# herobd/handwriting_line_generation

Hardware: AMD Instinct MI355X
Metric: G+D train steps/sec (higher is better)
Workload: dtype f32

## Files before the change

handwriting_line_generation_amd/csrc/conv_mfma.hip:

```cpp
#include "hwg_common.h"
#include "wino_pack.h"
#include <stdlib.h>

namespace {

struct ConvK {
  const float* x;
  const float* w;
  const float* bias;
  float* y;
  int N, H, W, C, K, R, S, sh, sw, ph, pw, dh, dw, P, Q;
  int mode;
  int KN;
  int Pm, Qm;
  int accumulate;
  int ntm;
  int ntm_pad;
  int nsplit;
  float* part;
  int* cnt;
  int dbg;
};

template <int BM, int BN, int BK, int WAVES_M, int WAVES_N, int PF = 1, int WK = 1, bool ABL = false>
// ... 567 lines not shown
    float af[2][PF][MI], bf[2][PF][NI];
    auto lds_group = [&](int g, int slot) {
#pragma unroll
      for (int u = 0; u < PF; ++u) {
        const int kk = kbeg + 2 * (g * PF + u) + lhi;
#pragma unroll
        for (int mi = 0; mi < MI; ++mi) af[slot][u][mi] = Ub[kk * BMU + wm0 + mi * 32 + l31];
#pragma unroll
        for (int ni = 0; ni < NI; ++ni) bf[slot][u][ni] = Vb[kk * BNV + wn0 + ni * 32 + l31];
      }
    };
    lds_group(0, 0);
#pragma unroll
    for (int g = 0; g < NG; ++g) {
      if (g + 1 < NG) lds_group(g + 1, (g + 1) & 1);
      __builtin_amdgcn_sched_barrier(0);
#pragma unroll
      for (int u = 0; u < PF; ++u)
#pragma unroll
        for (int mi = 0; mi < MI; ++mi)
#pragma unroll
          for (int ni = 0; ni < NI; ++ni)
            acc[mi][ni] = __builtin_amdgcn_mfma_f32_32x32x2f32(af[g & 1][u][mi], bf[g & 1][u][ni], acc[mi][ni], 0, 0, 0);
      __builtin_amdgcn_sched_barrier(0);
    }
    if (t + 1 < T) store_tile(buf ^ 1);
    __syncthreads();
  }

  if (do_bias && k0 + tid < a.K) a.part[(long long)blockIdx.x * a.pstride + (long long)RS * a.K * a.C + k0 + tid] = (float)bsum;

  if (WAVES_K > 1) {
    float* red = smem;
#pragma unroll
    for (int mi = 0; mi < MI; ++mi)
#pragma unroll
      for (int ni = 0; ni < NI; ++ni)
#pragma unroll
        for (int e = 0; e < 16; ++e) red[((wid * MI * NI + mi * NI + ni) * 16 + e) * 64 + lane] = acc[mi][ni][e];
    __syncthreads();
    if (wk != 0) return;
#pragma unroll
    for (int mi = 0; mi < MI; ++mi)
#pragma unroll
      for (int ni = 0; ni < NI; ++ni)
#pragma unroll
        for (int e = 0; e < 16; ++e) {
          float sacc = 0.f;
          for (int w = 0; w < WAVES_K; ++w) sacc += red[(((w * WMN + wmn) * MI * NI + mi * NI + ni) * 16 + e) * 64 + lane];
          acc[mi][ni][e] = sacc;
        }
  }

  float* pout = a.part + (long long)blockIdx.x * a.pstride + (long long)tap * a.K * a.C;
#pragma unroll
  for (int mi = 0; mi < MI; ++mi)
#pragma unroll
    for (int e = 0; e < 16; ++e) {
      const int k = k0 + wm0 + mi * 32 + (e & 3) + 8 * (e >> 2) + 4 * lhi;
      if (k >= a.K) continue;
#pragma unroll
      for (int ni = 0; ni < NI; ++ni) {
        const int c = c0 + wn0 + ni * 32 + l31;
        if (TAPN) {
          if (c < RS) pout[(long long)c * a.K + k] = acc[mi][ni][e];
        } else {
          if (c < a.C) pout[(long long)k * a.C + c] = acc[mi][ni][e];
        }
      }
    }
}

__device__ __forceinline__ void wgrad_reduce_vec4_body(const float* __restrict__ part, float* __restrict__ dw, int nsplit, int RS, int S, int K, int C,
                                                       long long sa, long long sb, long long sr, long long ss, int accumulate,
                                                       long long pstride, float* dbias, int bias_accumulate, int bid, int nb) {
  const long long total = (long long)RS * K * C;
  const long long all = total + (dbias ? K : 0);
  const long long n4 = all >> 2;
  for (long long j = bid * (long long)blockDim.x + threadIdx.x; j < n4; j += (long long)nb * blockDim.x) {
    const long long i = j << 2;
    float4 sum = *reinterpret_cast<const float4*>(part + i);
    int sp = 1;
    for (; sp + 3 < nsplit; sp += 4) {
      float4 v[4];
#pragma unroll
      for (int u = 0; u < 4; ++u) v[u] = *reinterpret_cast<const float4*>(part + (long long)(sp + u) * pstride + i);
#pragma unroll
      for (int u = 0; u < 4; ++u) { sum.x += v[u].x; sum.y += v[u].y; sum.z += v[u].z; sum.w += v[u].w; }
    }
    for (; sp < nsplit; ++sp) {
      const float4 v = *reinterpret_cast<const float4*>(part + (long long)sp * pstride + i);
      sum.x += v.x; sum.y += v.y; sum.z += v.z; sum.w += v.w;
    }
    const float e[4] = {sum.x, sum.y, sum.z, sum.w};
    if (i >= total) {
      const int k = (int)(i - total);
#pragma unroll
      for (int u = 0; u < 4; ++u) dbias[k + u] = bias_accumulate ? dbias[k + u] + e[u] : e[u];
      continue;
    }
    const unsigned iu = (unsigned)i, t = iu / (unsigned)C;
    const int c = (int)(iu - t * C);
    const int tap = (int)(t / (unsigned)K);
    const int k = (int)(t - (unsigned)tap * K);
    const long long o = k * sa + c * sb + (tap / S) * sr + (tap % S) * ss;
#pragma unroll
    for (int u = 0; u < 4; ++u) dw[o + u * sb] = accumulate ? dw[o + u * sb] + e[u] : e[u];
  }
}
__global__ __launch_bounds__(256) void wgrad_reduce_kernel(const float* __restrict__ part, float* __restrict__ dw, int nsplit, int RS, int S, int K, int C,
                                                           long long sa, long long sb, long long sr, long long ss, int accumulate,
                                                           long long pstride, float* dbias, int bias_accumulate) {
  wgrad_reduce_vec4_body(part, dw, nsplit, RS, S, K, C, sa, sb, sr, ss, accumulate, pstride, dbias, bias_accumulate, blockIdx.x, gridDim.x);
}
__device__ __forceinline__ void wgrad_reduce_scalar_body(const float* __restrict__ part, float* __restrict__ dw, int nsplit, int RS, int S, int K,
                                                         int C, long long sa, long long sb, long long sr, long long ss, int accumulate,
                                                         long long pstride, float* dbias, int bias_accumulate, int bid, int nb) {
  const long long total = (long long)RS * K * C;
  const long long all = total + (dbias ? K : 0);
  for (long long i = bid * (long long)blockDim.x + threadIdx.x; i < all; i += (long long)nb * blockDim.x) {
    float sum = 0.f;
    for (int sp = 0; sp < nsplit; ++sp) sum += part[(long long)sp * pstride + i];
    if (i >= total) {
      const int k = (int)(i - total);
      dbias[k] = bias_accumulate ? dbias[k] + sum : sum;
      continue;
    }
    const unsigned iu = (unsigned)i, t = iu / (unsigned)C;
    const int c = (int)(iu - t * C);
    const int tap = (int)(t / (unsigned)K);
    const int k = (int)(t - (unsigned)tap * K);
    const long long o = k * sa + c * sb + (tap / S) * sr + (tap % S) * ss;
    dw[o] = accumulate ? dw[o] + sum : sum;
  }
}
__global__ __launch_bounds__(256) void wgrad_reduce_scalar_kernel(const float* __restrict__ part, float* __restrict__ dw, int nsplit, int RS, int S, int K,
                                                                  int C, long long sa, long long sb, long long sr, long long ss, int accumulate,
                                                                  long long pstride, float* dbias, int bias_accumulate) {
  wgrad_reduce_scalar_body(part, dw, nsplit, RS, S, K, C, sa, sb, sr, ss, accumulate, pstride, dbias, bias_accumulate, blockIdx.x, gridDim.x);
}

template <int SL>
__device__ __forceinline__ void wgrad_reduce_lanes_body(const float* part, float* dw, int nsplit, int RS, int S, int K, int C,
                                                        long long sa, long long sb, long long sr, long long ss, int accumulate,
                                                        long long pstride, float* dbias, int bias_accumulate, int bid, float* red) {
  constexpr int OUT = 256 / SL;
  const long long total = (long long)RS * K * C;
  const long long all = total + (dbias ? K : 0);
  const int ol = threadIdx.x % OUT, lane = threadIdx.x / OUT;
  const long long i = (long long)bid * OUT + ol;
  float sum = 0.f;
  if (i < all) {
    int sp = lane;
    for (; sp + 3 * SL < nsplit; sp += 4 * SL) {
      const float v0 = part[(long long)sp * pstride + i], v1 = part[(long long)(sp + SL) * pstride + i];
      const float v2 = part[(long long)(sp + 2 * SL) * pstride + i], v3 = part[(long long)(sp + 3 * SL) * pstride + i];
      sum += v0; sum += v1; sum += v2; sum += v3;
    }
    for (; sp < nsplit; sp += SL) sum += part[(long long)sp * pstride + i];
  }
  red[lane * OUT + ol] = sum;
  __syncthreads();
  if (lane == 0 && i < all) {
    float t = 0.f;
#pragma unroll
    for (int l = 0; l < SL; ++l) t += red[l * OUT + ol];
    if (i >= total) {
      const int kb = (int)(i - total);
      dbias[kb] = bias_accumulate ? dbias[kb] + t : t;
      return;
    }
    const unsigned iu = (unsigned)i, q = iu / (unsigned)C;
    const int c = (int)(iu - q * C);
    const int tap = (int)(q / (unsigned)K);
    const int k = (int)(q - (unsigned)tap * K);
    const long long o = k * sa + c * sb + (tap / S) * sr + (tap % S) * ss;
    dw[o] = accumulate ? dw[o] + t : t;
  }
}
template <int SL>
__global__ __launch_bounds__(256) void wgrad_reduce_lanes_kernel(const float* part, float* dw, int nsplit, int RS, int S, int K, int C,
                                                                 long long sa, long long sb, long long sr, long long ss, int accumulate,
                                                                 long long pstride, float* dbias, int bias_accumulate) {
  __shared__ float red[256];
  wgrad_reduce_lanes_body<SL>(part, dw, nsplit, RS, S, K, C, sa, sb, sr, ss, accumulate, pstride, dbias, bias_accumulate, blockIdx.x, red);
}

template <int SL, int RSC>
__device__ __forceinline__ void wgrad_reduce_rows_body(const float* __restrict__ part, float* __restrict__ dw, int nsplit, int RS_rt, int K, int C,
                                                       long long sa, int accumulate, long long pstride, float* dbias, int bias_accumulate,
                                                       int main_blocks, int bid, float* red) {
  constexpr int KC = 256 / SL;
  const int RS = RSC ? RSC : RS_rt;
  const int ldp = RS | 1;
  const long long KCtot = (long long)K * C;
  if (bid >= main_blocks) {
    const int k = (bid - main_blocks) * 256 + threadIdx.x;
    if (k >= K) return;
    float s = 0.f;
    for (int sp = 0; sp < nsplit; ++sp) s += part[(long long)sp * pstride + RS * KCtot + k];
    dbias[k] = bias_accumulate ? dbias[k] + s : s;
    return;
  }
  const int pl = threadIdx.x % KC, sl = threadIdx.x / KC;
  const long long base = (long long)bid * KC;
  const long long kc = base + pl;
  if (kc < KCtot) {
    if (RSC) {
      float acc[RSC ? RSC : 1];
#pragma unroll
      for (int t = 0; t < RSC; ++t) acc[t] = 0.f;
      for (int sp = sl; sp < nsplit; sp += SL) {
        const float* src = part + (long long)sp * pstride + kc;
#pragma unroll
        for (int t = 0; t < RSC; ++t) acc[t] += src[t * KCtot];
      }
#pragma unroll
      for (int t = 0; t < RSC; ++t) red[(sl * KC + pl) * ldp + t] = acc[t];
    } else {
      for (int t = 0; t < RS; ++t) {
        float a = 0.f;
        for (int sp = sl; sp < nsplit; sp += SL) a += part[(long long)sp * pstride + t * KCtot + kc];
        red[(sl * KC + pl) * ldp + t] = a;
      }
    }
  }
  __syncthreads();
  const int n_out = KC * RS;
  for (int j = threadIdx.x; j < n_out; j += 256) {
    const int p = j / RS, t = j - p * RS;
    const long long q = base + p;
    if (q >= KCtot) break;
    float s = red[p * ldp + t];
#pragma unroll
    for (int l = 1; l < SL; ++l) s += red[(l * KC + p) * ldp + t];
    const long long k = q / C;
    const long long o = k * sa + (q - k * C) * RS + t;
    dw[o] = accumulate ? dw[o] + s : s;
  }
}
template <int SL, int RSC>
__global__ __launch_bounds__(256) void wgrad_reduce_rows_kernel(const float* __restrict__ part, float* __restrict__ dw, int nsplit, int RS_rt, int K, int C,
                                                                long long sa, int accumulate, long long pstride, float* dbias, int bias_accumulate,
                                                                int main_blocks) {
  extern __shared__ float red_rows[];
  wgrad_reduce_rows_body<SL, RSC>(part, dw, nsplit, RS_rt, K, C, sa, accumulate, pstride, dbias, bias_accumulate, main_blocks, blockIdx.x, red_rows);
}

enum { RED_VEC4 = 0, RED_SCALAR = 1, RED_LANES32 = 2, RED_LANES4 = 3, RED_ROWS = 4  };
struct RedEntry {
  const float* part; float* dw; float* dbias;
  long long pstride, sa, sb, sr, ss;
  int nsplit, RS, S, K, C, accumulate, bias_accumulate, variant, first_block, nblocks, main_blocks, tag;
};
constexpr int RED_MAX = 32;
struct RedTable { int n, pad; RedEntry e[RED_MAX]; };

__global__ __launch_bounds__(256) void wgrad_reduce_multi_kernel(const RedTable t) {
  extern __shared__ float red_multi[];
  int lo = 0, hi = t.n - 1;
  while (lo < hi) {
    const int mid = (lo + hi + 1) >> 1;
    if (t.e[mid].first_block <= (int)blockIdx.x) lo = mid; else hi = mid - 1;
  }
  const RedEntry& e = t.e[lo];
  const int bid = (int)blockIdx.x - e.first_block;
  switch (e.variant) {
    case RED_VEC4: wgrad_reduce_vec4_body(e.part, e.dw, e.nsplit, e.RS, e.S, e.K, e.C, e.sa, e.sb, e.sr, e.ss, e.accumulate, e.pstride, e.dbias, e.bias_accumulate, bid, e.nblocks); break;
    case RED_SCALAR: wgrad_reduce_scalar_body(e.part, e.dw, e.nsplit, e.RS, e.S, e.K, e.C, e.sa, e.sb, e.sr, e.ss, e.accumulate, e.pstride, e.dbias, e.bias_accumulate, bid, e.nblocks); break;
    case RED_LANES32: wgrad_reduce_lanes_body<32>(e.part, e.dw, e.nsplit, e.RS, e.S, e.K, e.C, e.sa, e.sb, e.sr, e.ss, e.accumulate, e.pstride, e.dbias, e.bias_accumulate, bid, red_multi); break;
    case RED_LANES4: wgrad_reduce_lanes_body<4>(e.part, e.dw, e.nsplit, e.RS, e.S, e.K, e.C, e.sa, e.sb, e.sr, e.ss, e.accumulate, e.pstride, e.dbias, e.bias_accumulate, bid, red_multi); break;
#define HWG_ROWS_CASE(ID, SL, RSC) \
    case RED_ROWS + ID: wgrad_reduce_rows_body<SL, RSC>(e.part, e.dw, e.nsplit, e.RS, e.K, e.C, e.sa, e.accumulate, e.pstride, e.dbias, e.bias_accumulate, e.main_blocks, bid, red_multi); break;
    HWG_ROWS_CASE(0, 1, 9) HWG_ROWS_CASE(1, 4, 9) HWG_ROWS_CASE(2, 1, 16) HWG_ROWS_CASE(3, 4, 16) HWG_ROWS_CASE(4, 1, 3) HWG_ROWS_CASE(5, 4, 3)
    HWG_ROWS_CASE(6, 1, 0) HWG_ROWS_CASE(7, 4, 0)
#undef HWG_ROWS_CASE
    default: break;
  }
}

__global__ void pack_weight_kernel(const float* src, float* dst, int A, int B, int Bpad, int R, int S,
                                   long long sa, long long sb, long long sr, long long ss, int flip) {
  const long long total = (long long)R * S * A * Bpad;
  for (long long i = blockIdx.x * (long long)blockDim.x + threadIdx.x; i < total; i += (long long)gridDim.x * blockDim.x) {
    const int b = (int)(i % Bpad);
    const long long t = i / Bpad;
    const int aa = (int)(t % A);
    const int tap = (int)(t / A);
    int r = tap / S, s = tap % S;
    if (flip) { r = R - 1 - r; s = S - 1 - s; }
    dst[i] = (b < B) ? src[aa * sa + b * sb + r * sr + s * ss] : 0.f;
  }
}

struct PackEntry {
  const float* src;
  float* dst;
  int A, B, Bpad, R, S, flip;
  long long sa, sb, sr, ss, total, first_block;
  int mode, Apad;
};

constexpr int PACK_PER_BLOCK = 1024;
__global__ __launch_bounds__(256) void pack_weight_multi_kernel(const PackEntry* table, int n) {
  int lo = 0, hi = n - 1;
  while (lo < hi) {
    const int mid = (lo + hi + 1) >> 1;
    if (table[mid].first_block <= (long long)blockIdx.x) lo = mid; else hi = mid - 1;
  }
  const PackEntry e = table[lo];
  const long long base = ((long long)blockIdx.x - e.first_block) * PACK_PER_BLOCK;
#pragma unroll
  for (int j = 0; j < PACK_PER_BLOCK / 256; ++j) {
    const long long i = base + j * 256 + threadIdx.x;
    if (i >= e.total) break;
    if (e.mode == 1) {
      wino_pack_one(e.src, e.dst, i, e.A, e.Apad, e.B, e.Bpad, e.sa, e.sb, e.sr, e.ss, e.flip);
      continue;
    }
    if (e.mode == 2) {
      wino_s2_pack_one(e.src, e.dst, i, e.A, e.B, e.sa, e.sb, e.flip);
      continue;
    }
    const int b = (int)(i % e.Bpad);
    const long long t = i / e.Bpad;
    const int aa = (int)(t % e.A);
    const int tap = (int)(t / e.A);
    int r = tap / e.S, s2 = tap % e.S;
    if (e.flip) { r = e.R - 1 - r; s2 = e.S - 1 - s2; }
    e.dst[i] = (b < e.B) ? e.src[aa * e.sa + b * e.sb + r * e.sr + s2 * e.ss] : 0.f;
  }
}

struct PackEntryS {
  PackEntry e;
  long long dst_off;
  int scale_idx, pad;
};
__global__ __launch_bounds__(256) void pack_weight_multi_scaled_kernel(const PackEntryS* table, int n, float* dst_base, const float* scale_base) {
  int lo = 0, hi = n - 1;
  while (lo < hi) {
    const int mid = (lo + hi + 1) >> 1;
    if (table[mid].e.first_block <= (long long)blockIdx.x) lo = mid; else hi = mid - 1;
  }
  const PackEntry e = table[lo].e;
  float* dst = dst_base + table[lo].dst_off;
  const float sc = scale_base[table[lo].scale_idx];
  const long long base = ((long long)blockIdx.x - e.first_block) * PACK_PER_BLOCK;
#pragma unroll
  for (int j = 0; j < PACK_PER_BLOCK / 256; ++j) {
    const long long i = base + j * 256 + threadIdx.x;
    if (i >= e.total) break;
    if (e.mode == 1) {
      wino_pack_one(e.src, dst, i, e.A, e.Apad, e.B, e.Bpad, e.sa, e.sb, e.sr, e.ss, e.flip, sc);
      continue;
    }
    if (e.mode == 2) {
      wino_s2_pack_one(e.src, dst, i, e.A, e.B, e.sa, e.sb, e.flip, sc);
      continue;
    }
    const int b = (int)(i % e.Bpad);
    const long long t = i / e.Bpad;
    const int aa = (int)(t % e.A);
    const int tap = (int)(t / e.A);
    int r = tap / e.S, s2 = tap % e.S;
    if (e.flip) { r = e.R - 1 - r; s2 = e.S - 1 - s2; }
    dst[i] = (b < e.B) ? __fmul_rn(e.src[aa * e.sa + b * e.sb + r * e.sr + s2 * e.ss], sc) : 0.f;
  }
}

template <int V>
__global__ __launch_bounds__(256) void colsum_partial_kernel(const float* x, long long rows, int C, float* part, long long rows_per_chunk,
                                                             float* direct_out, int accumulate) {
  __shared__ double red[256][V];
  const int cleft = C - (int)blockIdx.y * 64;
  const int cgn = V == 4 ? min(16, (cleft + 3) / 4) : min(64, cleft);
  const int RL = 256 / cgn;
  const int cg = threadIdx.x % cgn, rl = threadIdx.x / cgn;
  const int c = blockIdx.y * 64 + cg * V;
  const long long rb = blockIdx.x * rows_per_chunk;
  const long long re = min(rb + rows_per_chunk, rows);
  double s[V];
#pragma unroll
  for (int e = 0; e < V; ++e) s[e] = 0.0;
  if (rl < RL && c < C) {
    if (V == 4) {
      for (long long rr = rb + rl; rr < re; rr += 4ll * RL) {
        float4 v[4];
#pragma unroll
        for (int u = 0; u < 4; ++u) {
          const long long r2 = rr + (long long)u * RL;
          v[u] = *reinterpret_cast<const float4*>(x + (r2 < re ? r2 : rr) * C + c);
        }
#pragma unroll
        for (int u = 0; u < 4; ++u) {
          if (rr + (long long)u * RL >= re) break;
          s[0] += (double)v[u].x; s[1 % V] += (double)v[u].y; s[2 % V] += (double)v[u].z; s[3 % V] += (double)v[u].w;
        }
      }
    } else {
      for (long long rr = rb + rl; rr < re; rr += RL) s[0] += (double)x[rr * C + c];
    }
  }
#pragma unroll
  for (int e = 0; e < V; ++e) red[threadIdx.x][e] = s[e];
  __syncthreads();
  if ((int)threadIdx.x < min(64, cleft)) {
    const int cc = blockIdx.y * 64 + threadIdx.x;
    double v = 0.0;
    for (int r = 0; r < RL; ++r) v += red[r * cgn + (int)threadIdx.x / V][threadIdx.x % V];
    if (direct_out) direct_out[cc] = accumulate ? direct_out[cc] + (float)v : (float)v;
    else part[(long long)blockIdx.x * C + cc] = (float)v;
  }
}
template <int CC>
__global__ __launch_bounds__(256) void colsum_narrow_kernel(const float* __restrict__ x, long long rows, float* part, long long rows_per_chunk,
                                                            float* direct_out, int accumulate) {
  __shared__ double red[256][CC];
  const long long rb = blockIdx.x * rows_per_chunk;
  const long long re = min(rb + rows_per_chunk, rows);
  double s[CC];
#pragma unroll
  for (int c = 0; c < CC; ++c) s[c] = 0.0;
  for (long long r = rb + threadIdx.x; r < re; r += 256) {
#pragma unroll
    for (int c = 0; c < CC; ++c) s[c] += (double)x[r * CC + c];
  }
#pragma unroll
  for (int c = 0; c < CC; ++c) red[threadIdx.x][c] = s[c];
  __syncthreads();
  for (int w = 128; w >= 1; w >>= 1) {
    if ((int)threadIdx.x < w) {
#pragma unroll
      for (int c = 0; c < CC; ++c) red[threadIdx.x][c] += red[threadIdx.x + w][c];
    }
    __syncthreads();
  }
  if ((int)threadIdx.x < CC) {
    const float v = (float)red[0][threadIdx.x];
    if (direct_out) direct_out[threadIdx.x] = accumulate ? direct_out[threadIdx.x] + v : v;
    else part[(long long)blockIdx.x * CC + threadIdx.x] = v;
  }
}
__global__ __launch_bounds__(256) void colsum_final_kernel(const float* part, int chunks, int C, float* out, int accumulate) {
  __shared__ float red[16][17];
  const int cl = threadIdx.x & 15, lane = threadIdx.x >> 4;
  const int c = blockIdx.x * 16 + cl;
  float s = 0.f;
  if (c < C)
    for (int i = lane; i < chunks; i += 16) s += part[(long long)i * C + c];
  red[lane][cl] = s;
  __syncthreads();
  if (lane == 0 && c < C) {
    float t = 0.f;
#pragma unroll
    for (int l = 0; l < 16; ++l) t += red[l][cl];
    out[c] = accumulate ? out[c] + t : t;
  }
}

template <int BM, int BN, int BK, int WM_, int WN_>
void launch_conv(const ConvK& k, dim3 grid, hipStream_t st, int pf) {
  if constexpr (BM == 64 && BN == 64) {
    if (hwg_tune().conv_wk >= 2) {
      hipLaunchKernelGGL((conv_mfma_kernel<BM, BN, BK, WM_, WN_, 3, 2>), grid, dim3(128 * WM_ * WN_), 0, st, k);
      return;
    }
  }
  if constexpr (BM == 128 && BN == 128 && BK == 32) {
    if (k.dbg) { hipLaunchKernelGGL((conv_mfma_kernel<BM, BN, BK, WM_, WN_, 3, 1, true>), grid, dim3(64 * WM_ * WN_), 0, st, k); return; }
  }
  if (pf >= 3) hipLaunchKernelGGL((conv_mfma_kernel<BM, BN, BK, WM_, WN_, 3>), grid, dim3(64 * WM_ * WN_), 0, st, k);
  else if (pf == 2) hipLaunchKernelGGL((conv_mfma_kernel<BM, BN, BK, WM_, WN_, 2>), grid, dim3(64 * WM_ * WN_), 0, st, k);
  else hipLaunchKernelGGL((conv_mfma_kernel<BM, BN, BK, WM_, WN_, 1>), grid, dim3(64 * WM_ * WN_), 0, st, k);
}

struct WgPlan {
  int cfg;
  int bmu, bnv, bkp;
  int tiles_u, tiles_v, nsplit, chunk;
};
static void wg_split(WgPlan& p, long long Mtot, long long ns) {
  const long long max_ns = (Mtot + 4LL * p.bkp - 1) / (4LL * p.bkp);
  if (ns > max_ns) ns = max_ns;
  if (ns < 1) ns = 1;
  long long chunk = (Mtot + ns - 1) / ns;
  chunk = (chunk + p.bkp - 1) / p.bkp * p.bkp;
  ns = (Mtot + chunk - 1) / chunk;
  if (ns < 1) ns = 1;
  p.nsplit = (int)ns;
  p.chunk = (int)chunk;
}
static void wg_tile(WgPlan& p, int cfg, int K, int C) {
  p.cfg = cfg;
  if (cfg == 0) { p.bmu = 128; p.bnv = 128; p.bkp = 32; }
  else if (cfg == 1) { p.bmu = 64; p.bnv = 64; p.bkp = 32; }
  else { p.bmu = 32; p.bnv = 32; p.bkp = 32; }
  p.tiles_u = hwg_cdiv(K, p.bmu);
  p.tiles_v = hwg_cdiv(C, p.bnv);
}
static WgPlan plan_wgrad_model(const hwg_conv_desc* d);
WgPlan plan_wgrad(const hwg_conv_desc* d) {
  static thread_local HwgPlanCache<WgPlan> cache;
  return cache.get(d, plan_wgrad_model);
}
static WgPlan plan_wgrad_model(const hwg_conv_desc* d) {
  WgPlan p;
  const int K = d->K, C = d->C;
  const long long Mtot = (long long)d->N * d->P * d->Q;
  if (K <= 32 && C <= 32) {
    wg_tile(p, 2, K, C);
    const long long base = (long long)d->R * d->S * p.tiles_u * p.tiles_v;
    wg_split(p, Mtot, (1024 + base - 1) / base);
    return p;
  }
  if (const char* f = hwg_tune().wgrad_force; *f) {
    int fc = -1, ft = 0;
    if (sscanf(f, "%d,%d", &fc, &ft) == 2 && ft > 0 && (fc == 1 || (fc == 0 && K >= 128 && C >= 128))) {
      wg_tile(p, fc, K, C);
      const long long base = (long long)d->R * d->S * p.tiles_u * p.tiles_v;
      wg_split(p, Mtot, (ft + base - 1) / base);
      return p;
    }
  }
  static const int splits[14] = {1, 2, 3, 4, 6, 8, 12, 16, 24, 32, 48, 64, 96, 128};
  static const double tflops[2] = {106.0, 90.0}, overhead[2] = {1.0, 1.0};
  static const int waves_per_block[2] = {16, 8};
  const double wbytes = 4.0 * d->R * d->S * K * C;
  double best = 1e30;
  WgPlan bp = p;
  for (int cfg = (K >= 128 && C >= 128) ? 0 : 1; cfg <= 1; ++cfg) {
    WgPlan c;
    wg_tile(c, cfg, K, C);
    const double base = (double)d->R * d->S * c.tiles_u * c.tiles_v;
    int last_ns = 0;
    for (int si = 0; si < 14; ++si) {
      wg_split(c, Mtot, splits[si]);
      if (c.nsplit == last_ns) continue;
      last_ns = c.nsplit;
      if (wbytes * c.nsplit > 2.0e9) break;
      const double q = base * c.nsplit / 256.0;
      const double quanta = q <= 2.0 ? ceil(q) : q + 0.5;
      double resident = (q > 1.0 ? q : 1.0);
      const double max_blocks = 32.0 / waves_per_block[cfg];
      if (resident > max_blocks) resident = max_blocks;
      resident *= waves_per_block[cfg];
      const double rate = tflops[cfg] * (0.65 + 0.35 * (resident >= 24.0 ? 1.0 : resident / 24.0));
      const double step_s = 2.0 * c.bmu * c.bnv * c.bkp / (rate * 1e12 / 256.0);
      const double tm = quanta * ((double)c.chunk / c.bkp + overhead[cfg]) * step_s + (c.nsplit + 1) * wbytes / 8.0e12 + 3e-6;
      if (tm < best) { best = tm; bp = c; }
    }
  }
  return bp;
}

}

extern "C" int hwg_conv_pack_weight(const float* src, float* dst, int A, int B, int Bpad, int R, int S,
                                    long long sa, long long sb, long long sr, long long ss, int flip, void* stream) {
  HWG_REQUIRE(src && dst && A > 0 && B > 0 && Bpad >= B && R > 0 && S > 0, "conv_pack_weight: bad arguments");
  const long long total = (long long)R * S * A * Bpad;
  hipLaunchKernelGGL(pack_weight_kernel, dim3(hwg_stream_grid(total, 256)), dim3(256), 0, (hipStream_t)stream,
                     src, dst, A, B, Bpad, R, S, sa, sb, sr, ss, flip);
  HWG_LAUNCH_CHECK("conv_pack_weight");
  return HWG_OK;
}

extern "C" int hwg_conv_pack_weight_multi(const void* table, int n_entries, long long total_blocks, void* stream) {
  HWG_REQUIRE(table && n_entries > 0 && total_blocks > 0 && total_blocks < (1LL << 31), "conv_pack_weight_multi: bad arguments");
  hipLaunchKernelGGL(pack_weight_multi_kernel, dim3((unsigned)total_blocks), dim3(256), 0, (hipStream_t)stream, (const PackEntry*)table, n_entries);
  HWG_LAUNCH_CHECK("conv_pack_weight_multi");
  return HWG_OK;
}

extern "C" int hwg_conv_pack_weight_multi_scaled(const void* table, int n_entries, long long total_blocks, float* dst_base, const float* scale_base,
                                                 void* stream) {
  HWG_REQUIRE(table && dst_base && scale_base && n_entries > 0 && total_blocks > 0 && total_blocks < (1LL << 31), "conv_pack_weight_multi_scaled: bad arguments");
  hipLaunchKernelGGL(pack_weight_multi_scaled_kernel, dim3((unsigned)total_blocks), dim3(256), 0, (hipStream_t)stream, (const PackEntryS*)table, n_entries,
                     dst_base, scale_base);
  HWG_LAUNCH_CHECK("conv_pack_weight_multi_scaled");
  return HWG_OK;
}

int hwg_conv_c1_fwd_impl(const hwg_conv_desc* d, const float* x, const float* w, const float* bias, float* y, int accumulate, hipStream_t st);
int hwg_conv_to1_fwd_impl(const hwg_conv_desc* d, const float* x, const float* w, const float* bias, float* y, int accumulate, hipStream_t st);
int hwg_conv_wgrad_direct_impl(const hwg_conv_desc* d, const float* u, const float* v, float* dw, long long sa, long long sb,
                               long long sr, long long ss, int accumulate, void* ws, size_t ws_bytes, hipStream_t st);
size_t hwg_conv_wgrad_direct_workspace(const hwg_conv_desc* d);

static int check_desc(const hwg_conv_desc* d, const char* who) {
  HWG_REQUIRE(d, "%s: null descriptor", who);
  HWG_REQUIRE(d->N > 0 && d->H > 0 && d->W > 0 && d->C > 0 && d->K > 0 && d->R > 0 && d->S > 0 && d->P > 0 && d->Q > 0,
              "%s: non-positive dimension", who);
  HWG_REQUIRE(d->stride_h > 0 && d->stride_w > 0 && d->dil_h > 0 && d->dil_w > 0, "%s: bad stride/dilation", who);
  return HWG_OK;
}

int hwg_conv_split_reduce_launch(const float* part, const float* bias, float* y, long long total, int K, int nsplit, int accumulate, hipStream_t st) {
  hipLaunchKernelGGL(conv_split_reduce_kernel, dim3(hwg_stream_grid(total / 4 + 1, 256)), dim3(256), 0, st, part, bias, y, total, K, nsplit, accumulate);
  HWG_LAUNCH_CHECK("conv_split_reduce");
  return HWG_OK;
}

struct ConvPlan {
  bool mfma;
  int bm, bn, bk, nsplit, classes;
  long long Mc;
  int merged, KN, Pm, Qm;
  double model_s;
};
static ConvPlan plan_conv_model(const hwg_conv_desc* d);
static ConvPlan plan_conv(const hwg_conv_desc* d) {
  static thread_local HwgPlanCache<ConvPlan> cache;
  return cache.get(d, plan_conv_model);
}
static ConvPlan plan_conv_model(const hwg_conv_desc* d) {
  ConvPlan p;
  p.mfma = !((!d->transposed) && (d->K <= 2 || d->C == 1));
  p.classes = d->transposed ? d->stride_h * d->stride_w : 1;
  p.Mc = (long long)d->N * d->P * d->Q;
  if (d->transposed) p.Mc = (long long)d->N * hwg_cdiv(d->P, d->stride_h) * hwg_cdiv(d->Q, d->stride_w);
  p.merged = 0; p.KN = d->K; p.Pm = p.Qm = 0;
  if (d->transposed && p.classes > 1 && d->R % d->stride_h == 0 && d->S % d->stride_w == 0 &&
      (hwg_tune().conv_merge == 2 || (hwg_tune().conv_merge == 1 && d->K < 32))) {
    for (int c = 0; c < d->stride_h; ++c) p.Pm = std::max(p.Pm, hwg_cdiv(d->P - c, d->stride_h) + (c + d->pad_h) / d->stride_h);
    for (int c = 0; c < d->stride_w; ++c) p.Qm = std::max(p.Qm, hwg_cdiv(d->Q - c, d->stride_w) + (c + d->pad_w) / d->stride_w);
    p.merged = 1; p.KN = p.classes * d->K; p.Mc = (long long)d->N * p.Pm * p.Qm; p.classes = 1;
  }
  const int bk = (d->C % 32 == 0) ? 32 : 16;
  const int taps_total = d->R * d->S;
  const double taps_per_class = (double)taps_total / (d->transposed ? d->stride_h * d->stride_w : 1);
  const double T_total = taps_per_class * (d->C / bk);
  const int min_taps = d->transposed ? (d->R / d->stride_h) * (d->S / d->stride_w) : taps_total;
  const int min_steps = (min_taps > 0 ? min_taps : 1) * (d->C / bk);
  const double out_bytes = 4.0 * d->N * d->P * d->Q * d->K;
  struct Tile { int bm, bn; double tflops, overhead; };
  static const Tile tiles[4] = {{128, 128, 108.0, 1.0}, {128, 64, 94.0, 1.25}, {64, 64, 88.0, 1.5}, {128, 32, 62.0, 1.5}};
  static const int splits[8] = {1, 2, 3, 4, 6, 8, 12, 16};
  int bm = 128, bn = 32, ns = 1;
  double best = 1e30;
  for (int ti = 0; ti < 4; ++ti) {
    const Tile& t = tiles[ti];
    if (p.KN <= 32 ? t.bn != 32 : (t.bn == 32 || (t.bn == 128 && p.KN < 96))) continue;
    const double step_s = 2.0 * t.bm * t.bn * bk / (t.tflops * 1e12 / 256.0);
    const double per_xcd = (double)hwg_cdiv(hwg_cdiv(p.Mc, t.bm), 8) * hwg_cdiv(p.KN, t.bn) * p.classes;
    for (int si = 0; si < 8; ++si) {
      const int n = splits[si];
      if (n > 1 && (min_steps / n < 3 || out_bytes * n > 1.5e9)) break;
      const double q = per_xcd * n / 32.0;
      const double quanta = q <= 8.0 ? ceil(q) : q + 0.5;
// ... 727 lines not shown
```

handwriting_line_generation_amd/csrc/conv_wino.hip:

```cpp
#include "hwg_common.h"
#include "wino_pack.h"
#include <stdlib.h>

namespace {

struct WinoK {
  const float* x;
  const float* u;
  const float* bias;
  float* y;
  int N, H, W, C, K, Kpad, P, Q, ph, pw, TP, TQ;
  int M;
  int accumulate;
  int nsplit;
  float* part;
  int* cnt;
  int mt, nt;
  int xcd_order;
  int bal;
  int bal_tile0;
  int mt_edge;
  int dbg;
  int x_img, x_row, x_pix, x_tc, x_run;
  int y_img, y_row, y_pix, y_kc, y_run;
// ... 1137 lines not shown
  }
  if (!direct && a.cnt) {
    __shared__ int last_flag;
    if (hwg_split_arrive_block(a.cnt + slot_id, pieces, &last_flag)) {
      const long long total = (long long)a.N * a.P * a.Q * a.K;
      const int k = n0 + (tid & 63);
      const float bl = (a.bias && k < a.K) ? a.bias[k] : 0.f;
      auto finish = [&](long long o) {
        float v = BAL ? 0.f : hwg_load_agent(a.part + o);
        for (int sp = BAL ? 0 : 1; sp < pieces; ++sp) v += hwg_load_agent(a.part + sp * total + o);
        if (a.bias) v += bl;
        if (a.accumulate) v += a.y[o];
        a.y[o] = v;
      };
      if constexpr (MT == 2) {
        for (int tile = tid >> 6; tile < 64; tile += 8) {
          const int base = tile_out[tile], ext = tile_ext[tile];
          if (base < 0 || k >= a.K) continue;
          const long long ob = (long long)base * a.K + k;
#pragma unroll
          for (int i = 0; i < 2; ++i) {
            if (i && !(ext & 1)) continue;
#pragma unroll
            for (int j = 0; j < 2; ++j) {
              if (j && !(ext & 2)) continue;
              finish(ob + (i * a.Q + j) * a.K);
            }
          }
        }
      } else {
        const long long kch = (long long)(k / a.y_kc) * a.y_run + (k % a.y_kc);
        for (int tile = tid >> 6; tile < 64; tile += 8) {
          const int base = tile_out[tile], ext = tile_ext[tile];
          if (base < 0 || k >= a.K) continue;
          for (int i = 0; i < (ext & 3); ++i)
            for (int j = 0; j < (ext >> 2); ++j) finish((long long)base + (long long)i * a.y_row + (long long)j * a.y_pix + kch);
        }
      }
    }
  }
  if (!BAL || whole) break;
  unit += t1 - t0;
  if (unit >= unit_end) break;
  __syncthreads();
  }
}


constexpr int WINO_DB = 4;

__global__ __launch_bounds__(768) void wino_conv_big_kernel(WinoK a) {
  constexpr int TM = 64, TN = 64, NX = 256;
  constexpr int PSV = TM * 16 + 8, PSU = TN * 16 + 8;
  constexpr int VBUF = 4 * PSV, UBUF = 4 * PSU;
  constexpr int DA = WINO_DB;
  constexpr int XI = TM * 16 / NX;
  constexpr int UD = TN / 16;
  __shared__ __attribute__((aligned(16))) float smem[2 * VBUF + DA * UBUF];
  float* const Vs = smem;
  float* const Us = smem + 2 * VBUF;

  const int tid = threadIdx.x, lane = tid & 63, wid = tid >> 6;
  int mtile, ntile, split;
  if (!wino_work_item(a, mtile, ntile, split)) return;
  const int m0 = mtile * TM;
  const int n0 = ntile * TN;
  const int T_all = a.C >> 4;
  const int t0 = (int)((long long)T_all * split / a.nsplit);
  const int t1 = (int)((long long)T_all * (split + 1) / a.nsplit);
  const int S = 4 * (t1 - t0);
  const int TC = t1 - t0;
  const int rot = TC > 0 ? (int)(((unsigned)mtile * 7u + (unsigned)ntile * 3u) % (unsigned)TC) : 0;
  auto chunk_of = [&](int tau) { int c = tau + rot; if (c >= TC) c -= TC; return t0 + c; };

  if (wid >= 8) {
    const int pt = tid - 512;
    const int pw = wid - 8;
    int x_off[XI], x_ok[XI];
    const int xb = pt & 3, xc4 = (pt >> 2) & 3;
    const int x_lds0 = xb * PSV + swz(pt >> 4, xc4);
    const float x_sa = (xb == 3) ? -1.f : 1.f, x_sb = (xb & 1) ? 1.f : -1.f;
    const int row_stride = a.W * a.C;
#pragma unroll
    for (int it = 0; it < XI; ++it) {
      const int b = xb, c4 = xc4, row = (pt >> 4) + 16 * it;
      const int m = m0 + row;
      const bool mok = m < a.M;
      const int mm = mok ? m : 0;
      const int tj = mm % a.TQ;
      const int t2 = mm / a.TQ;
      const int ti = t2 % a.TP;
      const int n = t2 / a.TP;
      const int w = 2 * tj - a.pw + b;
      const bool wok = mok && w >= 0 && w < a.W;
      const int h0 = 2 * ti - a.ph;
      x_off[it] = ((n * a.H + h0) * a.W + (wok ? w : 0)) * a.C + c4 * 4;
      int okm = 0;
#pragma unroll
      for (int r = 0; r < 4; ++r)
        if (wok && h0 + r >= 0 && h0 + r < a.H) okm |= 1 << r;
      x_ok[it] = okm;
    }
    int u_src[UD];
#pragma unroll
    for (int i = 0; i < UD; ++i) {
      const int row = 16 * i + (lane >> 2), slot = lane & 3;
      int k = n0 + row;
      if (k >= a.Kpad) k = a.Kpad - 1;
      u_src[i] = (pw * a.Kpad + k) * 16 + 4 * (slot ^ ((row >> 1) & 3));
    }
    const long long u_round = 4LL * a.Kpad * 16;
    float4 raw[XI][4], tr[XI][4];
    auto load_x = [&](int t) {
#pragma unroll
      for (int it = 0; it < XI; ++it)
#pragma unroll
        for (int r = 0; r < 4; ++r) {
          const int off = (x_ok[it] >> r) & 1 ? x_off[it] + r * row_stride + t * 16 : 0;
          raw[it][r] = *reinterpret_cast<const float4*>(a.x + off);
        }
    };
    auto col_transform = [&]() {
#pragma unroll
      for (int it = 0; it < XI; ++it) {
        float4 d[4];
#pragma unroll
        for (int r = 0; r < 4; ++r) {
          d[r] = raw[it][r];
          if (!((x_ok[it] >> r) & 1)) d[r] = make_float4(0.f, 0.f, 0.f, 0.f);
        }
        tr[it][0] = make_float4(d[0].x - d[2].x, d[0].y - d[2].y, d[0].z - d[2].z, d[0].w - d[2].w);
        tr[it][1] = make_float4(d[1].x + d[2].x, d[1].y + d[2].y, d[1].z + d[2].z, d[1].w + d[2].w);
        tr[it][2] = make_float4(d[2].x - d[1].x, d[2].y - d[1].y, d[2].z - d[1].z, d[2].w - d[1].w);
        tr[it][3] = make_float4(d[1].x - d[3].x, d[1].y - d[3].y, d[1].z - d[3].z, d[1].w - d[3].w);
      }
    };
    auto dma_u = [&](int ring, int round) {
      const float* base = a.u + (long long)round * u_round;
      float* dst = Us + ring * UBUF + pw * PSU;
#pragma unroll
      for (int i = 0; i < UD; ++i)
        __builtin_amdgcn_global_load_lds((const __attribute__((address_space(1))) void*)(base + u_src[i]),
                                         (__attribute__((address_space(3))) void*)(dst + i * 256), 16, 0, 0);
    };
    auto write_v = [&](int buf, int r) {
      float* B = Vs + buf * VBUF;
#pragma unroll
      for (int it = 0; it < XI; ++it) {
        const float4 v = tr[it][r];
        float4 o;
        o.x = x_sa * v.x + x_sb * quad_partner(v.x);
        o.y = x_sa * v.y + x_sb * quad_partner(v.y);
        o.z = x_sa * v.z + x_sb * quad_partner(v.z);
        o.w = x_sa * v.w + x_sb * quad_partner(v.w);
        *reinterpret_cast<float4*>(B + x_lds0 + it * 256) = o;
      }
    };
    int hist[DA], hdma[DA];
#pragma unroll
    for (int j = 0; j < DA; ++j) { hist[j] = 0; hdma[j] = 0; }
    int issued = 0;
    if (S > 0) {
      load_x(chunk_of(0));
      col_transform();
      write_v(0, 0);
    }
    for (; issued < DA && issued < S; ++issued) dma_u(issued, 4 * chunk_of(issued >> 2) + (issued & 3));
    wait_vmcnt((issued - 1) * UD);
#pragma unroll
    for (int j = 0; j < DA; ++j) { hdma[j] = j < issued ? UD : 0; hist[j] = hdma[j]; }
    __syncthreads();
    int ring = 0;
    for (int t = t0; t < t1; ++t) {
#pragma unroll
      for (int r = 0; r < 4; ++r) {
        const int s = 4 * (t - t0) + r;
        int ops = 0, dops = 0;
        if (s >= 1 && issued < S) { dma_u(ring, 4 * chunk_of(issued >> 2) + (issued & 3)); ++issued; ring = ring == DA - 1 ? 0 : ring + 1; ops = dops = UD; }
        if (s + 1 < S) {
          if (r == 3) col_transform();
          write_v((r + 1) & 1, (r + 1) & 3);
          if (r == 1 && t + 1 < t1) { load_x(chunk_of(t + 1 - t0)); ops += XI * 4; }
        }
#pragma unroll
        for (int j = 0; j + 1 < DA; ++j) { hist[j] = hist[j + 1]; hdma[j] = hdma[j + 1]; }
        hist[DA - 1] = ops; hdma[DA - 1] = dops;
        if (s + 1 < S) {
          int back = issued - 2 - s;
          int n = 0, seen = 0;
#pragma unroll
          for (int j = DA - 1; j >= 0; --j) {
            if (seen < back || (seen == back && hdma[j] == 0)) { n += hist[j]; seen += hdma[j] ? 1 : 0; }
            else if (seen == back && hdma[j] != 0) { n += hist[j] - hdma[j]; seen = back + 1; }
          }
          wait_vmcnt(n);
        }
        __syncthreads();
      }
    }
    return;
  }

  const int cm = wid >> 2, cn = wid & 3;
  const int frow = lane & 15, fchunk = lane >> 4;
  const int a_off0 = swz(cm * 32 + frow, fchunk);
  const int a_off1 = swz(cm * 32 + 16 + frow, fchunk);
  const int b_off = swz(cn * 16 + frow, fchunk);

  f32x4 acc[16][2];
#pragma unroll
  for (int p = 0; p < 16; ++p) {
    acc[p][0] = (f32x4){0.f, 0.f, 0.f, 0.f};
    acc[p][1] = (f32x4){0.f, 0.f, 0.f, 0.f};
  }
  __syncthreads();
  int ring = 0;
  for (int t = t0; t < t1; ++t) {
#pragma unroll
    for (int r = 0; r < 4; ++r) {
      const float* A = Vs + (r & 1) * VBUF;
      const float* B = Us + ring * UBUF + b_off;
      ring = ring == DA - 1 ? 0 : ring + 1;
      float4 fa0[2], fa1[2], fb[2];
      fa0[0] = *reinterpret_cast<const float4*>(A + a_off0);
      fa1[0] = *reinterpret_cast<const float4*>(A + a_off1);
      fb[0] = *reinterpret_cast<const float4*>(B);
#pragma unroll
      for (int pb = 0; pb < 4; ++pb) {
        const int c = pb & 1;
        if (pb < 3) {
          fa0[c ^ 1] = *reinterpret_cast<const float4*>(A + (pb + 1) * PSV + a_off0);
          fa1[c ^ 1] = *reinterpret_cast<const float4*>(A + (pb + 1) * PSV + a_off1);
          fb[c ^ 1] = *reinterpret_cast<const float4*>(B + (pb + 1) * PSU);
        }
        __builtin_amdgcn_sched_barrier(0);
        f32x4& c0 = acc[r * 4 + pb][0];
        f32x4& c1 = acc[r * 4 + pb][1];
        c0 = __builtin_amdgcn_mfma_f32_16x16x4f32(fa0[c].x, fb[c].x, c0, 0, 0, 0);
        c1 = __builtin_amdgcn_mfma_f32_16x16x4f32(fa1[c].x, fb[c].x, c1, 0, 0, 0);
        c0 = __builtin_amdgcn_mfma_f32_16x16x4f32(fa0[c].y, fb[c].y, c0, 0, 0, 0);
        c1 = __builtin_amdgcn_mfma_f32_16x16x4f32(fa1[c].y, fb[c].y, c1, 0, 0, 0);
        c0 = __builtin_amdgcn_mfma_f32_16x16x4f32(fa0[c].z, fb[c].z, c0, 0, 0, 0);
        c1 = __builtin_amdgcn_mfma_f32_16x16x4f32(fa1[c].z, fb[c].z, c1, 0, 0, 0);
        c0 = __builtin_amdgcn_mfma_f32_16x16x4f32(fa0[c].w, fb[c].w, c0, 0, 0, 0);
        c1 = __builtin_amdgcn_mfma_f32_16x16x4f32(fa1[c].w, fb[c].w, c1, 0, 0, 0);
        __builtin_amdgcn_sched_barrier(0);
      }
      __syncthreads();
    }
  }

  const int k = n0 + cn * 16 + (lane & 15);
  const bool direct = a.nsplit == 1;
  float* yg = direct ? a.y : a.part + (long long)split * ((long long)a.N * a.P * a.Q * a.K);
  const float bv = (direct && a.bias && k < a.K) ? a.bias[k] : 0.f;
  const bool accum = direct && a.accumulate;
#pragma unroll
  for (int blk = 0; blk < 2; ++blk)
#pragma unroll
    for (int e = 0; e < 4; ++e) {
      const int m = m0 + cm * 32 + blk * 16 + (lane >> 4) * 4 + e;
      if (m >= a.M || k >= a.K) continue;
      const int tj = m % a.TQ;
      const int t2 = m / a.TQ;
      const int ti = t2 % a.TP;
      const int n = t2 / a.TP;
      float mm[16];
#pragma unroll
      for (int p = 0; p < 16; ++p) mm[p] = acc[p][blk][e];
#pragma unroll
      for (int j = 0; j < 4; ++j) {
        const float s0 = mm[0 * 4 + j] + mm[1 * 4 + j] + mm[2 * 4 + j];
        const float s1 = mm[1 * 4 + j] - mm[2 * 4 + j] - mm[3 * 4 + j];
        mm[0 * 4 + j] = s0;
        mm[1 * 4 + j] = s1;
      }
#pragma unroll
      for (int i = 0; i < 2; ++i) {
        const int p = 2 * ti + i;
        if (p >= a.P) continue;
        const float y0 = mm[i * 4 + 0] + mm[i * 4 + 1] + mm[i * 4 + 2];
        const float y1 = mm[i * 4 + 1] - mm[i * 4 + 2] - mm[i * 4 + 3];
#pragma unroll
        for (int j = 0; j < 2; ++j) {
          const int q = 2 * tj + j;
          if (q >= a.Q) continue;
          const long long o = (((long long)n * a.P + p) * a.Q + q) * a.K + k;
          float v = (j == 0 ? y0 : y1) + bv;
          if (accum) v += yg[o];
          yg[o] = v;
        }
      }
    }
}

__global__ __launch_bounds__(256) void wino_pack_weight_kernel(const float* src, float* dst, int A, int Apad, int B, int Bpad,
                                                               long long sa, long long sb, long long sr, long long ss, int flip) {
  const long long total = (long long)Apad * Bpad;
  for (long long i = blockIdx.x * (long long)blockDim.x + threadIdx.x; i < total; i += (long long)gridDim.x * blockDim.x)
    wino_pack_one(src, dst, i, A, Apad, B, Bpad, sa, sb, sr, ss, flip);
}

template <int VEC>
__global__ __launch_bounds__(256) void wino_bal_reduce_kernel(WinoK a, int T_all) {
  const int KV = a.K / VEC;
  const int total = a.N * a.P * a.Q * KV;
  const long long plane = (long long)a.N * a.P * a.Q * a.K;
  const int U_bal = (a.mt * a.nt - a.bal_tile0) * T_all;
  const int e = a.mt_edge;
  for (int i = blockIdx.x * blockDim.x + threadIdx.x; i < total; i += gridDim.x * blockDim.x) {
    const int k = (i % KV) * VEC, pix = i / KV;
    const int q = pix % a.Q, t = pix / a.Q, p = t % a.P, n = t / a.P;
    const int m = (n * a.TP + p / e) * a.TQ + q / e;
    const int rel = (m >> 6) + a.mt * (k >> 6) - a.bal_tile0;
    if (rel < 0) continue;
    const int g_first = wino_bal_owner(a.bal, U_bal, rel * T_all), g_last = wino_bal_owner(a.bal, U_bal, rel * T_all + T_all - 1);
    if (g_first == g_last) continue;
    const long long o = (long long)n * a.y_img + (long long)p * a.y_row + (long long)q * a.y_pix + (long long)(k / a.y_kc) * a.y_run + k % a.y_kc;
    float s[VEC];
#pragma unroll
    for (int v = 0; v < VEC; ++v) s[v] = 0.f;
    for (int j = 0; j <= g_last - g_first; ++j) {
      if constexpr (VEC == 4) {
        const float4 v = *reinterpret_cast<const float4*>(a.part + j * plane + o);
        s[0] += v.x; s[1] += v.y; s[2] += v.z; s[3] += v.w;
      } else {
        s[0] += a.part[j * plane + o];
      }
    }
#pragma unroll
    for (int v = 0; v < VEC; ++v) {
      if (a.bias) s[v] += a.bias[k + v];
      if (a.accumulate) s[v] += a.y[o + v];
    }
    if constexpr (VEC == 4) *reinterpret_cast<float4*>(a.y + o) = make_float4(s[0], s[1], s[2], s[3]);
    else a.y[o] = s[0];
  }
}

struct WinoPlan {
  int cfg;
  int tm, tn, nsplit;
  int bal, bal_tile0, bal_pieces;
  int bal_segs, bal_cut, bal_cut_pieces;
  double model_s;
};
static void wino_cfg(WinoPlan& p, int cfg) {
  static const int tms[8] = {64, 32, 128, 64, 32, 64, 64, 32}, tns[8] = {32, 64, 16, 32, 64, 64, 64, 32};
  p.cfg = cfg; p.tm = tms[cfg]; p.tn = tns[cfg];
  p.bal = p.bal_tile0 = p.bal_pieces = p.bal_segs = p.bal_cut = p.bal_cut_pieces = 0;
}
static bool wino_balance(WinoPlan& p, long long tiles, int chunks, int g_force = 0, int a_force = -1) {
  const long long lead = a_force >= 0 ? (long long)a_force : tiles / 256 * 256;
  const long long rem = tiles - lead;
  if (lead % 256 || rem <= 0 || (g_force <= 0 && rem >= 240)) return false;
  const long long units = rem * chunks;
  long long G = g_force > 0 ? g_force : (units < 256 ? units : 256);
  if (G > units) G = units;
  if (G < 1 || (g_force <= 0 && G <= rem) || units * G >= (1ll << 31) || units >= (1ll << 24)) return false;
  p.bal = (int)G; p.bal_tile0 = (int)lead; p.nsplit = 1;
  p.bal_pieces = 1; p.bal_segs = 1; p.bal_cut = 0; p.bal_cut_pieces = 0;
  for (long long t = 0; t < rem; ++t) {
    const int n = wino_bal_owner((int)G, (int)units, (int)(t * chunks + chunks - 1)) - wino_bal_owner((int)G, (int)units, (int)(t * chunks)) + 1;
    if (n > p.bal_pieces) p.bal_pieces = n;
    if (n > 1) { ++p.bal_cut; p.bal_cut_pieces += n; }
  }
  for (long long g = 0; g < G; ++g) {
    const long long u0 = units * g / G, u1 = units * (g + 1) / G;
    if (u1 > u0) p.bal_segs = std::max(p.bal_segs, (int)((u1 - 1) / chunks - u0 / chunks + 1));
  }
  return true;
}
struct WinoCost { int cfg; double fixed_us, step_us; };
static const WinoCost kWinoCost[6] = {{1, 2.5, 1.17}, {5, 11.0, 2.09}, {0, 8.0, 1.2}, {2, 6.5, 1.5}, {6, 15.7, 1.04}, {7, 2.0, 1.0}};
static WinoPlan plan_wino_model(const hwg_conv_desc* d);
static WinoPlan plan_wino(const hwg_conv_desc* d, double* model_s = nullptr) {
  static thread_local HwgPlanCache<WinoPlan> cache;
  const WinoPlan p = cache.get(d, plan_wino_model);
  if (model_s) *model_s = p.model_s;
  return p;
}
static WinoPlan plan_wino_model(const hwg_conv_desc* d) {
  WinoPlan best;
  wino_cfg(best, d->K <= 16 ? 2 : d->K <= 48 ? 0 : 1);
  best.nsplit = 1;
  const long long M = (long long)d->N * hwg_cdiv(d->P, 2) * hwg_cdiv(d->Q, 2);
  const int chunks = d->C / 16;
  const double out_bytes = 4.0 * d->N * d->P * d->Q * d->K;
  double best_t = 1e30;
  WinoCost cost6 = kWinoCost[4];
  if (const char* e = hwg_tune().wino_cost6; *e) { double f = 0, s2 = 0; if (sscanf(e, "%lf,%lf", &f, &s2) == 2) { cost6.fixed_us = f; cost6.step_us = s2; } }
  for (int ci = 0; ci < 6; ++ci) {
    const WinoCost& wc = ci == 4 ? cost6 : kWinoCost[ci];
    if (wc.cfg == 7 && (d->K <= 16 || d->K > 64)) continue;
    if (wc.cfg == 2 && d->K > 16) continue;
    if (wc.cfg == 0 && d->K > 48) continue;
    if ((wc.cfg == 1 || wc.cfg == 5 || wc.cfg == 6) && d->K <= 48) continue;
    if (wc.cfg == 5 && d->C < 64) continue;
    WinoPlan p;
    wino_cfg(p, wc.cfg);
    const long long blocks = (long long)hwg_cdiv(M, p.tm) * hwg_cdiv(d->K, p.tn);
    for (int ns = 1; ns <= 8 && ns * 2 <= (chunks > 1 ? chunks : 2); ns *= 2) {
      if (ns > 1 && (chunks / ns < 2 || out_bytes * ns > 1.5e9)) break;
      const double q = (double)(blocks * ns) / 256.0;
      const double rounds = q <= 3.0 ? (double)hwg_cdiv(blocks * ns, 256) : q + 0.5;
      double t = rounds * (wc.fixed_us + 4.0 * hwg_cdiv(chunks, ns) * wc.step_us) * 1e-6;
      if (ns > 1) t += (ns + 1) * out_bytes / 3.0e12 + 6e-6;
      if (t < best_t) { best_t = t; best = p; best.nsplit = ns; }
    }
  }
  const int bal_mode = hwg_tune().wino_bal[0] ? atoi(hwg_tune().wino_bal) : 0;
  if (d->K > 48 && bal_mode >= 0 && !hwg_tune().w64_nodma && !(hwg_tune().conv_dbg & 512) && (long long)d->N * d->P * d->Q * d->K < (1ll << 31)) {
    WinoPlan p;
    wino_cfg(p, 6);
    const long long tiles = (long long)hwg_cdiv(M, 64) * hwg_cdiv(d->K, 64);
    int gf = 0, af = -1;
    if (bal_mode > 0) sscanf(hwg_tune().wino_bal, "%d,%d", &gf, &af);
    if (wino_balance(p, tiles, chunks, gf, af) && (p.bal_pieces <= 1 || (double)p.bal_pieces * out_bytes <= 1.5e9)) {
      const long long units = (tiles - p.bal_tile0) * chunks;
      const long long c = hwg_cdiv(units, (long long)p.bal);
      double t = (p.bal_tile0 / 256) * (cost6.fixed_us + 4.0 * chunks * cost6.step_us) * 1e-6;
      t += (double)hwg_cdiv((long long)p.bal, 256ll) * (cost6.fixed_us - 4.0 + (p.bal_segs - 1) * 5.0 + 4.0 * c * cost6.step_us) * 1e-6;
      if (p.bal_cut) t += (p.bal_cut_pieces + p.bal_cut) * (out_bytes / tiles) / 3.0e12 + out_bytes / 2.0e13 + 6e-6;
      if (bal_mode > 0 || t < 0.97 * best_t) { best = p; best_t = t; }
    }
  }
  if (const char* f = hwg_tune().wino_force; *f) {
    int fc = -1, fs = 0;
    const int n = sscanf(f, "%d,%d", &fc, &fs);
    if (n >= 1 && fc >= 0 && fc <= 7 && fc != 3 && fc != 4 && (fc == 2 || d->K > 16)) { const int ns = best.nsplit; wino_cfg(best, fc); best.nsplit = ns; }
    if (n >= 2 && fs >= 1) best.nsplit = fs > chunks ? chunks : fs;
  }
  best.model_s = best_t;
  return best;
}

}

extern "C" int hwg_wino_supported(const hwg_conv_desc* d) {
  if (!d || d->transposed) return 0;
  if (d->R != 3 || d->S != 3 || d->stride_h != 1 || d->stride_w != 1 || d->dil_h != 1 || d->dil_w != 1) return 0;
  if (d->C % 16 != 0 || d->K < 16) return 0;
  if (d->P != d->H + 2 * d->pad_h - 2 || d->Q != d->W + 2 * d->pad_w - 2) return 0;
  return hwg_tune().wino == 0 ? 0 : 1;
}

double hwg_conv_direct_model_seconds(const hwg_conv_desc* d);

extern "C" int hwg_wino_preferred(const hwg_conv_desc* d) {
  if (!hwg_wino_supported(d)) return 0;
  if (hwg_tune().wino == 2) return 1;
  double tw = 0.0;
  (void)plan_wino(d, &tw);
  return tw < 0.97 * hwg_conv_direct_model_seconds(d) ? 1 : 0;
}

extern "C" size_t hwg_wino_weight_floats(int A, int B) {
  const size_t Apad = (size_t)(A + 15) / 16 * 16, Bpad = (size_t)(B + 15) / 16 * 16;
  return 16 * Apad * Bpad;
}

extern "C" int hwg_wino_pack_weight(const float* src, float* dst, int A, int B, long long sa, long long sb, long long sr, long long ss,
                                    int flip, void* stream) {
  HWG_REQUIRE(src && dst && A > 0 && B > 0, "wino_pack_weight: bad arguments");
  const int Apad = (A + 15) / 16 * 16, Bpad = (B + 15) / 16 * 16;
  hipLaunchKernelGGL(wino_pack_weight_kernel, dim3(hwg_stream_grid((long long)Apad * Bpad, 256)), dim3(256), 0, (hipStream_t)stream, src, dst, A, Apad,
                     B, Bpad, sa, sb, sr, ss, flip);
  HWG_LAUNCH_CHECK("wino_pack_weight");
  return HWG_OK;
}

extern "C" size_t hwg_wino_conv_workspace(const hwg_conv_desc* d) {
  if (!hwg_wino_supported(d)) return 0;
  const WinoPlan p = plan_wino(d);
  if (p.bal > 0) return p.bal_pieces > 1 ? (size_t)p.bal_pieces * d->N * d->P * d->Q * d->K * sizeof(float) : 0;
  if (p.nsplit <= 1) return 0;
  return (size_t)p.nsplit * d->N * d->P * d->Q * d->K * sizeof(float);
}

int hwg_conv_split_reduce_launch(const float* part, const float* bias, float* y, long long total, int K, int nsplit, int accumulate, hipStream_t st);

extern "C" int hwg_wino_conv_fwd(const hwg_conv_desc* d, const float* x, const float* u, const float* bias, float* y, int accumulate,
                                 void* workspace, size_t workspace_bytes, void* stream) {
  HWG_REQUIRE(d && x && u && y, "wino_conv_fwd: null pointer");
  HWG_REQUIRE(hwg_wino_supported(d), "wino_conv_fwd: needs a 3x3 stride-1 dilation-1 convolution with C %% 16 == 0 and K >= 16");
  hipStream_t st = (hipStream_t)stream;
  const WinoPlan p = plan_wino(d);
  const size_t need = hwg_wino_conv_workspace(d);
  if (need && (!workspace || workspace_bytes < need)) {
    hwg_set_error("wino_conv_fwd: workspace too small (%zu < %zu)", workspace_bytes, need);
    return HWG_ERR_WORKSPACE;
  }
  WinoK k;
  k.x = x; k.u = u; k.bias = bias; k.y = y;
  k.N = d->N; k.H = d->H; k.W = d->W; k.C = d->C; k.K = d->K; k.Kpad = (d->K + 15) / 16 * 16;
  k.P = d->P; k.Q = d->Q; k.ph = d->pad_h; k.pw = d->pad_w;
  k.TP = hwg_cdiv(d->P, 2); k.TQ = hwg_cdiv(d->Q, 2);
  k.M = d->N * k.TP * k.TQ;
  k.accumulate = accumulate;
  k.nsplit = p.nsplit;
  k.part = (float*)workspace;
  k.mt = hwg_cdiv(k.M, p.tm); k.nt = hwg_cdiv(d->K, p.tn);
  k.xcd_order = hwg_tune().wino_order;
  k.bal = p.bal; k.bal_tile0 = p.bal_tile0;
  k.mt_edge = 2; k.dbg = hwg_tune().conv_dbg;
  k.x_img = k.x_row = k.x_pix = k.x_tc = k.x_run = 0;
  k.y_img = d->P * d->Q * d->K; k.y_row = d->Q * d->K; k.y_pix = d->K; k.y_kc = d->K; k.y_run = 0;
  dim3 grid(p.bal > 0 ? p.bal_tile0 + (p.bal + 7) / 8 * 8 : (k.mt * k.nt * p.nsplit + 7) / 8 * 8);
  k.cnt = nullptr;
  const bool counted = p.cfg == 0 || p.cfg == 1 || p.cfg == 2 || p.cfg == 7 || (p.cfg == 6 && !hwg_tune().w64_nodma && !(hwg_tune().conv_dbg & 512));
  if ((p.bal > 0 ? p.bal_pieces > 1 : p.nsplit > 1) && counted && hwg_tune().split_inkernel && (long long)k.mt * k.nt * 8 <= HWG_SPLIT_COUNTERS) {
    k.cnt = hwg_split_counters(st);
    if (!k.cnt) return HWG_ERR_LAUNCH;
  }
  const int prof = hwg_prof_open(HWG_PROF_CONV_WINO, 2.0 * d->N * d->P * d->Q * (double)d->K * d->C * 9.0, st);
  if (p.cfg == 0) hipLaunchKernelGGL((wino_conv_kernel<4, 2>), grid, dim3(512), 0, st, k);
  else if (p.cfg == 1) hipLaunchKernelGGL((wino_conv_kernel<2, 4>), grid, dim3(512), 0, st, k);
  else if (p.cfg == 2) hipLaunchKernelGGL((wino_conv_kernel<8, 1>), grid, dim3(512), 0, st, k);
  else if (p.cfg == 7) hipLaunchKernelGGL((wino_conv_kernel<2, 2>), grid, dim3(256), 0, st, k);
  else if (p.cfg == 5) hipLaunchKernelGGL(wino_conv_big_kernel, grid, dim3(768), 0, st, k);
  else if (p.cfg == 6 && !hwg_tune().w64_nodma && (hwg_tune().conv_dbg & 512)) hipLaunchKernelGGL((wino_conv64d_kernel<1, false>), grid, dim3(512), 0, st, k);
  else if (p.cfg == 6 && !hwg_tune().w64_nodma && p.bal > 0) hipLaunchKernelGGL((wino_conv64d_kernel<0, true>), grid, dim3(512), 0, st, k);
  else if (p.cfg == 6 && !hwg_tune().w64_nodma) hipLaunchKernelGGL((wino_conv64d_kernel<0, false>), grid, dim3(512), 0, st, k);
  else if (p.cfg == 6) hipLaunchKernelGGL(wino_conv64_kernel, grid, dim3(512), 0, st, k);
  else hipLaunchKernelGGL((wino_conv_ws_kernel<1, 4>), grid, dim3(512), 0, st, k);
  hwg_prof_close(prof, st);
  hwg_note_plan(HWG_PROF_CONV_WINO, p.cfg, p.bal > 0 ? -p.bal : p.nsplit);
  HWG_LAUNCH_CHECK("wino_conv_fwd");
  if (k.cnt) {
  } else if (p.bal > 0 && p.bal_pieces > 1) {
    const long long total = (long long)d->N * d->P * d->Q * d->K;
    const double cut = (double)(k.mt * k.nt - p.bal_tile0) / (k.mt * k.nt);
    const int prof2 = hwg_prof_open(HWG_PROF_CONV_REDUCE, 4.0 * total * cut * (p.bal_pieces + 1), st);
    const int vec = d->K % 4 == 0 ? 4 : 1;
    const dim3 rgrid(hwg_stream_grid(total / vec, 256));
    if (vec == 4) hipLaunchKernelGGL(wino_bal_reduce_kernel<4>, rgrid, dim3(256), 0, st, k, d->C / 16);
    else hipLaunchKernelGGL(wino_bal_reduce_kernel<1>, rgrid, dim3(256), 0, st, k, d->C / 16);
    hwg_prof_close(prof2, st);
    HWG_LAUNCH_CHECK("wino_bal_reduce");
  } else if (p.nsplit > 1) {
    const long long total = (long long)d->N * d->P * d->Q * d->K;
    const int prof2 = hwg_prof_open(HWG_PROF_CONV_REDUCE, 4.0 * total * (p.nsplit + 1), st);
    const int rc = hwg_conv_split_reduce_launch((const float*)workspace, bias, y, total, d->K, p.nsplit, accumulate, st);
    hwg_prof_close(prof2, st);
    if (rc) return rc;
  }
  return HWG_OK;
}


namespace {

struct S2Geom {
  int N, Hv, Wv, Cv, Kv, Pv, Qv, pad;
  int x_img, x_row, x_pix, x_tc, x_run, y_img, y_row, y_pix, y_kc, y_run;
  double flops;
};

bool s2_geom(const hwg_conv_desc* d, S2Geom& g) {
  if (!d || d->R != 4 || d->S != 4 || d->stride_h != 2 || d->stride_w != 2 || d->pad_h || d->pad_w || d->dil_h != 1 || d->dil_w != 1) return false;
  if (d->C % 16 || d->K % 4 || d->N < 1 || d->H < 1 || d->W < 1) return false;
  const long long in_e = (long long)d->N * d->H * d->W * d->C, out_e = (long long)d->N * d->P * d->Q * d->K;
  if (in_e >= (1ll << 31) || out_e >= (1ll << 31)) return false;
  g.N = d->N;
  if (!d->transposed) {
    if (d->H < 4 || d->W < 4 || d->P != (d->H - 4) / 2 + 1 || d->Q != (d->W - 4) / 2 + 1) return false;
    g.Hv = d->P + 1; g.Wv = d->Q + 1; g.Cv = 4 * d->C; g.Kv = d->K; g.Pv = d->P; g.Qv = d->Q; g.pad = 0;
    g.x_img = d->H * d->W * d->C; g.x_row = 2 * d->W * d->C; g.x_pix = 2 * d->C; g.x_tc = 2 * d->C / 16; g.x_run = d->W * d->C;
    g.y_img = d->P * d->Q * d->K; g.y_row = d->Q * d->K; g.y_pix = d->K; g.y_kc = d->K; g.y_run = 0;
    g.flops = 2.0 * d->N * d->P * d->Q * (double)d->K * d->C * 16.0;
  } else {
    if (d->P != 2 * d->H + 2 || d->Q != 2 * d->W + 2) return false;
    g.Hv = d->H; g.Wv = d->W; g.Cv = d->C; g.Kv = 4 * d->K; g.Pv = d->H + 1; g.Qv = d->W + 1; g.pad = 1;
    g.x_img = d->H * d->W * d->C; g.x_row = d->W * d->C; g.x_pix = d->C; g.x_tc = d->C / 16; g.x_run = 0;
    g.y_img = d->P * d->Q * d->K; g.y_row = 2 * d->Q * d->K; g.y_pix = 2 * d->K; g.y_kc = 2 * d->K; g.y_run = d->Q * d->K;
    g.flops = 2.0 * d->N * d->H * d->W * (double)d->K * d->C * 16.0;
  }
  return g.Kv > 48;
}

WinoPlan plan_wino_s2_model(const hwg_conv_desc* d) {
  WinoPlan best;
  wino_cfg(best, 6);
  best.nsplit = 1;
  best.model_s = 1e30;
  S2Geom g;
  if (!s2_geom(d, g)) return best;
  const long long M = (long long)g.N * hwg_cdiv(g.Pv, 3) * hwg_cdiv(g.Qv, 3);
  const int chunks = g.Cv / 16;
  const double out_bytes = 4.0 * g.N * g.Pv * g.Qv * g.Kv;
  const WinoCost wc = kWinoCost[4];
  const long long tiles = (long long)hwg_cdiv(M, 64) * hwg_cdiv(g.Kv, 64);
  double best_t = 1e30;
  for (int ns = 1; ns <= 8 && ns * 2 <= (chunks > 1 ? chunks : 2); ns *= 2) {
    if (ns > 1 && (chunks / ns < 2 || out_bytes * ns > 1.5e9)) break;
    const double q = (double)(tiles * ns) / 256.0;
    const double rounds = q <= 3.0 ? (double)hwg_cdiv(tiles * ns, 256) : q + 0.5;
    double t = rounds * (wc.fixed_us + 4.0 * hwg_cdiv(chunks, ns) * wc.step_us) * 1e-6;
    if (ns > 1) t += (ns + 1) * out_bytes / 3.0e12 + 6e-6;
    if (t < best_t) { best_t = t; best.nsplit = ns; }
  }
  const int bal_mode = hwg_tune().wino_bal[0] ? atoi(hwg_tune().wino_bal) : 0;
  if (bal_mode >= 0) {
    WinoPlan p;
    wino_cfg(p, 6);
    int gf = 0, af = -1;
    if (bal_mode > 0) sscanf(hwg_tune().wino_bal, "%d,%d", &gf, &af);
    if (wino_balance(p, tiles, chunks, gf, af) && (p.bal_pieces <= 1 || (double)p.bal_pieces * out_bytes <= 1.5e9)) {
      const long long units = (tiles - p.bal_tile0) * chunks;
      const long long c = hwg_cdiv(units, (long long)p.bal);
      double t = (p.bal_tile0 / 256) * (wc.fixed_us + 4.0 * chunks * wc.step_us) * 1e-6;
      t += (double)hwg_cdiv((long long)p.bal, 256ll) * (wc.fixed_us - 4.0 + (p.bal_segs - 1) * 5.0 + 4.0 * c * wc.step_us) * 1e-6;
      if (p.bal_cut) t += (p.bal_cut_pieces + p.bal_cut) * (out_bytes / tiles) / 3.0e12 + out_bytes / 2.0e13 + 6e-6;
      if (bal_mode > 0 || t < 0.97 * best_t) { best = p; best_t = t; }
    }
  }
  if (const char* f = hwg_tune().wino_force; *f) {
    int fc = -1, fs = 0;
    if (sscanf(f, "%d,%d", &fc, &fs) >= 2 && fs >= 1) { const int keep = fs > chunks ? chunks : fs; wino_cfg(best, 6); best.nsplit = keep; }
  }
  best.model_s = best_t;
  return best;
}
WinoPlan plan_wino_s2(const hwg_conv_desc* d) {
  static thread_local HwgPlanCache<WinoPlan> cache;
  return cache.get(d, plan_wino_s2_model);
}

__global__ __launch_bounds__(256) void wino_s2_pack_kernel(const float* src, float* dst, int Kc, int Cc, long long sk, long long sc, int dgrad, long long total) {
  for (long long i = blockIdx.x * (long long)blockDim.x + threadIdx.x; i < total; i += (long long)gridDim.x * blockDim.x)
    wino_s2_pack_one(src, dst, i, Kc, Cc, sk, sc, dgrad);
}

}

extern "C" int hwg_wino_s2_supported(const hwg_conv_desc* d) {
  S2Geom g;
  return hwg_tune().wino_s2 != 0 && !hwg_tune().w64_nodma && s2_geom(d, g) ? 1 : 0;
}

extern "C" int hwg_wino_s2_preferred(const hwg_conv_desc* d) {
  if (!hwg_wino_s2_supported(d)) return 0;
  if (hwg_tune().wino_s2 == 2) return 1;
  const WinoPlan p = plan_wino_s2(d);
  return p.model_s < 0.9 * hwg_conv_direct_model_seconds(d) ? 1 : 0;
}

extern "C" size_t hwg_wino_s2_weight_floats(int Kc, int Cc, int dgrad) {
  const size_t A = dgrad ? 4 * (size_t)Cc : (size_t)Kc, B = dgrad ? (size_t)Kc : 4 * (size_t)Cc;
  return 16 * ((A + 15) / 16 * 16) * ((B + 15) / 16 * 16);
}

extern "C" int hwg_wino_s2_pack_weight(const float* src, float* dst, int Kc, int Cc, long long sk, long long sc, int dgrad, void* stream) {
  HWG_REQUIRE(src && dst && Kc > 0 && Cc > 0, "wino_s2_pack_weight: bad arguments");
  const long long total = (long long)hwg_wino_s2_weight_floats(Kc, Cc, dgrad) / 16;
  hipLaunchKernelGGL(wino_s2_pack_kernel, dim3(hwg_stream_grid(total, 256)), dim3(256), 0, (hipStream_t)stream, src, dst, Kc, Cc, sk, sc, dgrad, total);
  HWG_LAUNCH_CHECK("wino_s2_pack_weight");
  return HWG_OK;
}

extern "C" size_t hwg_wino_s2_workspace(const hwg_conv_desc* d) {
  if (!hwg_wino_s2_supported(d)) return 0;
  const WinoPlan p = plan_wino_s2(d);
  const size_t out = (size_t)d->N * d->P * d->Q * d->K * sizeof(float);
  if (p.bal > 0) return p.bal_pieces > 1 ? p.bal_pieces * out : 0;
  return p.nsplit > 1 ? p.nsplit * out : 0;
}

extern "C" int hwg_wino_s2_conv(const hwg_conv_desc* d, const float* x, const float* u, const float* bias, float* y, int accumulate,
                                void* workspace, size_t workspace_bytes, void* stream) {
  HWG_REQUIRE(d && x && u && y, "wino_s2_conv: null pointer");
  S2Geom g;
  HWG_REQUIRE(hwg_wino_s2_supported(d) && s2_geom(d, g), "wino_s2_conv: needs a 4x4 stride-2 pad-0 convolution (or its data gradient) with C %% 16 == 0");
  HWG_REQUIRE(!(d->transposed && bias), "wino_s2_conv: the data-gradient form takes no bias");
  hipStream_t st = (hipStream_t)stream;
  const WinoPlan p = plan_wino_s2(d);
  const size_t need = hwg_wino_s2_workspace(d);
  if (need && (!workspace || workspace_bytes < need)) {
    hwg_set_error("wino_s2_conv: workspace too small (%zu < %zu)", workspace_bytes, need);
    return HWG_ERR_WORKSPACE;
  }
  WinoK k;
  k.x = x; k.u = u; k.bias = bias; k.y = y;
  k.N = g.N; k.H = g.Hv; k.W = g.Wv; k.C = g.Cv; k.K = g.Kv; k.Kpad = (g.Kv + 15) / 16 * 16;
  k.P = g.Pv; k.Q = g.Qv; k.ph = g.pad; k.pw = g.pad;
  k.TP = hwg_cdiv(g.Pv, 3); k.TQ = hwg_cdiv(g.Qv, 3);
  k.M = g.N * k.TP * k.TQ;
  k.accumulate = accumulate;
  k.nsplit = p.nsplit;
  k.part = (float*)workspace;
  k.mt = hwg_cdiv(k.M, 64); k.nt = hwg_cdiv(g.Kv, 64);
  k.xcd_order = hwg_tune().wino_order;
  k.bal = p.bal; k.bal_tile0 = p.bal_tile0;
  k.mt_edge = 3; k.dbg = 0;
  k.x_img = g.x_img; k.x_row = g.x_row; k.x_pix = g.x_pix; k.x_tc = g.x_tc; k.x_run = g.x_run;
  k.y_img = g.y_img; k.y_row = g.y_row; k.y_pix = g.y_pix; k.y_kc = g.y_kc; k.y_run = g.y_run;
  dim3 grid(p.bal > 0 ? p.bal_tile0 + (p.bal + 7) / 8 * 8 : (k.mt * k.nt * p.nsplit + 7) / 8 * 8);
  k.cnt = nullptr;
  if ((p.bal > 0 ? p.bal_pieces > 1 : p.nsplit > 1) && hwg_tune().split_inkernel && (long long)k.mt * k.nt <= HWG_SPLIT_COUNTERS) {
    k.cnt = hwg_split_counters(st);
    if (!k.cnt) return HWG_ERR_LAUNCH;
  }
  const int prof = hwg_prof_open(HWG_PROF_CONV_WINO, g.flops, st);
  if (p.bal > 0) hipLaunchKernelGGL((wino_conv64d_kernel<0, true, 3>), grid, dim3(512), 0, st, k);
  else hipLaunchKernelGGL((wino_conv64d_kernel<0, false, 3>), grid, dim3(512), 0, st, k);
  hwg_prof_close(prof, st);
  hwg_note_plan(HWG_PROF_CONV_WINO, 36, p.bal > 0 ? -p.bal : p.nsplit);
  HWG_LAUNCH_CHECK("wino_s2_conv");
  const long long total = (long long)d->N * d->P * d->Q * d->K;
  if (k.cnt) {
  } else if (p.bal > 0 && p.bal_pieces > 1) {
    const double cut = (double)(k.mt * k.nt - p.bal_tile0) / (k.mt * k.nt);
    const int prof2 = hwg_prof_open(HWG_PROF_CONV_REDUCE, 4.0 * total * cut * (p.bal_pieces + 1), st);
    hipLaunchKernelGGL(wino_bal_reduce_kernel<4>, dim3(hwg_stream_grid(total / 4, 256)), dim3(256), 0, st, k, g.Cv / 16);
    hwg_prof_close(prof2, st);
    HWG_LAUNCH_CHECK("wino_bal_reduce");
  } else if (p.bal <= 0 && p.nsplit > 1) {
    const int prof2 = hwg_prof_open(HWG_PROF_CONV_REDUCE, 4.0 * total * (p.nsplit + 1), st);
    const int rc = hwg_conv_split_reduce_launch((const float*)workspace, bias, y, total, d->K, p.nsplit, accumulate, st);
    hwg_prof_close(prof2, st);
    if (rc) return rc;
  }
  return HWG_OK;
}

extern "C" int hwg_wino_conv_describe(const hwg_conv_desc* d, int* out) {
  HWG_REQUIRE(d && out, "wino_conv_describe: null pointer");
  for (int i = 0; i < 8; ++i) out[i] = -1;
  WinoPlan p;
  long long tiles;
  int chunks;
  S2Geom g;
  if (d->R == 4 && d->S == 4) {
    if (!hwg_wino_s2_supported(d) || !s2_geom(d, g)) return HWG_OK;
    p = plan_wino_s2(d);
    tiles = (long long)hwg_cdiv((long long)g.N * hwg_cdiv(g.Pv, 3) * hwg_cdiv(g.Qv, 3), 64ll) * hwg_cdiv(g.Kv, 64);
    chunks = g.Cv / 16;
  } else {
    if (!hwg_wino_supported(d)) return HWG_OK;
    p = plan_wino(d);
    tiles = (long long)hwg_cdiv((long long)d->N * hwg_cdiv(d->P, 2) * hwg_cdiv(d->Q, 2), (long long)p.tm) * hwg_cdiv(d->K, p.tn);
    chunks = d->C / 16;
  }
  out[0] = p.cfg; out[1] = p.nsplit; out[2] = p.bal; out[3] = p.bal_tile0; out[4] = p.bal > 0 ? p.bal_pieces : (p.nsplit > 1 ? p.nsplit : 1);
  out[5] = (int)tiles; out[6] = chunks; out[7] = p.bal > 0 ? p.bal_segs : 1;
  return HWG_OK;
}
```

handwriting_line_generation_amd/csrc/seq_ops.hip:

```cpp
#include "hwg_common.h"

namespace {

__global__ __launch_bounds__(256) void log_softmax_fwd_kernel(const float* x, float* y, long long rows, int C, int Bn, int Tn, int transpose) {
  const int lane = threadIdx.x & 63;
  const long long wave = (blockIdx.x * 256LL + threadIdx.x) >> 6;
  const long long nw = (gridDim.x * 256LL) >> 6;
  for (long long r = wave; r < rows; r += nw) {
    const float* xr = x + r * C;
    float m = -INFINITY;
    for (int c = lane; c < C; c += 64) m = fmaxf(m, xr[c]);
    m = wave_max(m);
    float s = 0.f;
    for (int c = lane; c < C; c += 64) s += expf(xr[c] - m);
    s = wave_sum(s);
    const float lse = m + logf(s);
    long long orow = r;
    if (transpose) { const long long b = r / Tn, t = r % Tn; orow = t * Bn + b; }
    float* yr = y + orow * C;
    for (int c = lane; c < C; c += 64) yr[c] = xr[c] - lse;
  }
}
__global__ __launch_bounds__(256) void log_softmax_bwd_kernel(const float* dy, const float* y, float* dx, long long rows, int C, int Bn, int Tn,
                                                              int transpose) {
  const int lane = threadIdx.x & 63;
  const long long wave = (blockIdx.x * 256LL + threadIdx.x) >> 6;
  const long long nw = (gridDim.x * 256LL) >> 6;
  for (long long r = wave; r < rows; r += nw) {
    long long orow = r;
    if (transpose) { const long long b = r / Tn, t = r % Tn; orow = t * Bn + b; }
    const float* dyr = dy + orow * C;
    const float* yr = y + orow * C;
    float s = 0.f;
    for (int c = lane; c < C; c += 64) s += dyr[c];
    s = wave_sum(s);
    float* dxr = dx + r * C;
    for (int c = lane; c < C; c += 64) dxr[c] = dyr[c] - expf(yr[c]) * s;
  }
}

__device__ __forceinline__ int ctc_ext(const int* tg, int s) { return (s & 1) ? tg[s >> 1] : 0; }

__device__ __forceinline__ void ctc_alpha_body(float* rows , int b, const float* lp,
                                               const int* targets, const int* in_len, const int* tg_len, int T, int B, int C, int Lmax,
                                               float* log_alpha, float* nll) {
  const int S = tg_len[b];
  const int Tb = in_len[b];
  const int NS = 2 * S + 1;
  const int NSmax = 2 * Lmax + 1;
  const int* tg = targets + (long long)b * Lmax;
  float* la = log_alpha + (long long)b * T * NSmax;
  int* ext = (int*)(rows + 2 * NSmax);
  const float NEG = -INFINITY;
  for (int s = threadIdx.x; s < NSmax; s += 256) {
    float v = NEG;
    if (Tb > 0) {
      if (s == 0) v = lp[((long long)0 * B + b) * C + 0];
      else if (s == 1 && S > 0) v = lp[((long long)0 * B + b) * C + tg[0]];
    }
    la[s] = v;
    rows[s] = v;
    ext[s] = s < NS ? ctc_ext(tg, s) : 0;
  }
  __syncthreads();
  for (int t = 1; t < Tb; ++t) {
    const float* prev = rows + ((t - 1) & 1) * NSmax;
    float* cur = rows + (t & 1) * NSmax;
    for (int s = threadIdx.x; s < NSmax; s += 256) {
      float v = NEG;
      if (s < NS) {
        const int cs = ext[s];
        const float l = lp[((long long)t * B + b) * C + cs];
        const float la1 = prev[s];
        float lamax = la1;
        float la2 = NEG, la3 = NEG;
        if (s > 0) { la2 = prev[s - 1]; if (la2 > lamax) lamax = la2; }
        if (s > 1 && ext[s - 2] != cs) { la3 = prev[s - 2]; if (la3 > lamax) lamax = la3; }
        if (lamax == NEG) lamax = 0.f;
        v = logf(expf(la1 - lamax) + expf(la2 - lamax) + expf(la3 - lamax)) + lamax + l;
      }
      cur[s] = v;
      la[(long long)t * NSmax + s] = v;
    }
    __syncthreads();
  }
  if (threadIdx.x == 0) {
    float r;
    if (Tb <= 0) r = (S == 0) ? 0.f : INFINITY;
    else {
      const float* last = rows + ((Tb - 1) & 1) * NSmax;
      const float l1 = last[NS - 1];
      const float l2 = (S > 0) ? last[NS - 2] : NEG;
      float m = fmaxf(l1, l2);
      if (m == NEG) m = 0.f;
      r = -(logf(expf(l1 - m) + expf(l2 - m)) + m);
    }
    nll[b] = r;
  }
}
__global__ __launch_bounds__(256) void ctc_alpha_kernel(const float* lp, const int* targets, const int* in_len, const int* tg_len, int T, int B,
                                                        int C, int Lmax, float* log_alpha, float* nll) {
  extern __shared__ float rows[];
  ctc_alpha_body(rows, blockIdx.x, lp, targets, in_len, tg_len, T, B, C, Lmax, log_alpha, nll);
}
__global__ void ctc_mean_kernel(const float* nll, const int* tg_len, int B, float* loss, int* finite_flag) {
  if (threadIdx.x == 0 && blockIdx.x == 0) {
    float s = 0.f;
    for (int b = 0; b < B; ++b) { const int l = tg_len[b] > 1 ? tg_len[b] : 1; s += nll[b] / (float)l; }
    s /= (float)B;
    const int inf = isinf(s) ? 1 : 0;
    *finite_flag = inf ? 0 : 1;
    *loss = inf ? 0.f : s;
  }
}
__device__ __forceinline__ void ctc_beta_body(float* rows , int b, const float* lp,
                                              const int* targets, const int* in_len, const int* tg_len, int T, int B, int C, int Lmax,
                                              float* log_beta) {
  const int S = tg_len[b];
  const int Tb = in_len[b];
  const int NS = 2 * S + 1;
  const int NSmax = 2 * Lmax + 1;
  const int* tg = targets + (long long)b * Lmax;
  float* lb = log_beta + (long long)b * T * NSmax;
  int* ext = (int*)(rows + 2 * NSmax);
  const float NEG = -INFINITY;
  for (int s = threadIdx.x; s < NSmax; s += 256) ext[s] = s < NS ? ctc_ext(tg, s) : 0;
  __syncthreads();
  if (Tb <= 0) return;
  for (int t = Tb - 1; t >= 0; --t) {
    float* cur = rows + (t & 1) * NSmax;
    const float* nxt = rows + ((t + 1) & 1) * NSmax;
    for (int s = threadIdx.x; s < NSmax; s += 256) {
      float v = NEG;
      if (s < NS) {
        const int cs = ext[s];
        const float l = lp[((long long)t * B + b) * C + cs];
        if (t == Tb - 1) {
          if (s == NS - 1 || (S > 0 && s == NS - 2)) v = l;
        } else {
          const float lb1 = nxt[s];
          float lbmax = lb1;
          float lb2 = NEG, lb3 = NEG;
          if (s < NS - 1) { lb2 = nxt[s + 1]; if (lb2 > lbmax) lbmax = lb2; }
          if (s < NS - 2 && ext[s + 2] != cs) { lb3 = nxt[s + 2]; if (lb3 > lbmax) lbmax = lb3; }
          if (lbmax == NEG) lbmax = 0.f;
          v = logf(expf(lb1 - lbmax) + expf(lb2 - lbmax) + expf(lb3 - lbmax)) + lbmax + l;
        }
      }
      cur[s] = v;
      lb[(long long)t * NSmax + s] = v;
    }
    __syncthreads();
  }
}
__global__ __launch_bounds__(256) void ctc_beta_kernel(const float* lp, const int* targets, const int* in_len, const int* tg_len, int T, int B,
                                                       int C, int Lmax, float* log_beta) {
  extern __shared__ float rows[];
  ctc_beta_body(rows, blockIdx.x, lp, targets, in_len, tg_len, T, B, C, Lmax, log_beta);
}
__global__ __launch_bounds__(256) void ctc_alpha_beta_kernel(const float* lp, const int* targets, const int* in_len, const int* tg_len, int T, int B,
                                                             int C, int Lmax, float* log_alpha, float* nll, float* log_beta) {
  extern __shared__ float rows[];
  if ((int)blockIdx.x < B) ctc_alpha_body(rows, blockIdx.x, lp, targets, in_len, tg_len, T, B, C, Lmax, log_alpha, nll);
  else ctc_beta_body(rows, blockIdx.x - B, lp, targets, in_len, tg_len, T, B, C, Lmax, log_beta);
}

__global__ __launch_bounds__(128) void ctc_grad_kernel(const float* lp, const int* targets, const int* in_len, const int* tg_len, int T, int B, int C,
                                                       int Lmax, const float* log_alpha, const float* log_beta, const float* nll, const float* grad_out,
                                                       const int* finite_flag, float* grad) {
  extern __shared__ float ab[];
  const int t = blockIdx.x, b = blockIdx.y;
  const int S = tg_len[b];
  const int Tb = in_len[b];
  const int NS = 2 * S + 1;
  const int NSmax = 2 * Lmax + 1;
  float* g = grad + ((long long)t * B + b) * C;
  if (t >= Tb) {
    for (int c = threadIdx.x; c < C; c += 128) g[c] = 0.f;
    return;
  }
  const int* tg = targets + (long long)b * Lmax;
  int* ext = (int*)(ab + NSmax);
  const long long row = ((long long)b * T + t) * NSmax;
  for (int s = threadIdx.x; s < NS; s += 128) {
    ab[s] = log_alpha[row + s] + log_beta[row + s];
    ext[s] = ctc_ext(tg, s);
  }
  __syncthreads();
  const float NEG = -INFINITY;
  const float nl = nll[b];
  const int tl = S > 1 ? S : 1;
  const float gr = (*finite_flag) ? grad_out[0] / ((float)tl * (float)B) : 0.f;
  const bool bad = !(*finite_flag) || isinf(nl);
  const float* lpr = lp + ((long long)t * B + b) * C;
  for (int c = threadIdx.x; c < C; c += 128) {
    float m = NEG;
    for (int s = (c == 0 ? 0 : 1); s < NS; s += 2)
      if (ext[s] == c && ab[s] > m) m = ab[s];
    float sum = 0.f;
    if (m != NEG)
      for (int s = (c == 0 ? 0 : 1); s < NS; s += 2)
        if (ext[s] == c && ab[s] != NEG) sum += expf(ab[s] - m);
    const float acc = (sum > 0.f) ? logf(sum) + m : NEG;
    const float l = lpr[c];
    float v = (expf(l) - expf(acc + nl - l)) * gr;
    if (bad) v = 0.f;
    g[c] = v;
  }
}

__global__ __launch_bounds__(256) void dtw_kernel(const float* pred, const int* label, int T, int B, int C, int L, unsigned char* history,
                                                  int* path, long long* out, int* lens) {
  extern __shared__ float diag[];
  const int b = blockIdx.x;
  const int LL = 2 * L + 1;
  const int w = max(T / 2, abs(T - LL));
  float* d0 = diag;
  float* d1 = diag + (LL + 1);
  float* d2 = diag + 2 * (LL + 1);
  const float INF = INFINITY;
  unsigned char* hist = history + (long long)b * T * LL;
  for (int j = threadIdx.x; j <= LL; j += 256) { d0[j] = INF; d1[j] = INF; d2[j] = INF; }
  __syncthreads();
  if (threadIdx.x == 0) d1[0] = 0.f;
  __syncthreads();
  for (int d = 1; d <= T + LL; ++d) {
    for (int j = threadIdx.x; j <= LL; j += 256) {
      const int i = d - j;
      float v = INF;
      if (i >= 1 && i <= T && j >= 1) {
        const int jlo = max(1, i - w), jhi = min(LL, i + w);
        if (j >= jlo && j <= jhi) {
          const int lab = ((j - 1) & 1) ? label[((j - 1) >> 1) * B + b] : 0;
          const float cost = 1.f - pred[((long long)(i - 1) * B + b) * C + lab];
          const float up = d1[j];
          const float dg = d0[j - 1];
          const float lf = d1[j - 1];
          float m = up; int h = 0;
          if (dg < m) { m = dg; h = 1; }
          if (lf < m) { m = lf; h = 2; }
          v = cost + m;
          hist[(long long)(i - 1) * LL + (j - 1)] = (unsigned char)h;
        }
      }
      d2[j] = v;
    }
    __syncthreads();
    float* tmp = d0; d0 = d1; d1 = d2; d2 = tmp;
  }
  __shared__ int s_len;
  int* pb = path + (long long)b * (T + LL);
  if (threadIdx.x == 0) {
    int i = T - 1, j = LL - 1, n = 0;
    pb[n++] = (j & 1) ? label[(j >> 1) * B + b] : 0;
    while ((i > 0 || j > 0) && n < T + LL) {
      const int h = hist[(long long)i * LL + j];
      if (h == 0) { if (i > 0) i -= 1; else j -= 1; }
      else if (h == 1) { if (i > 0) i -= 1; if (j > 0) j -= 1; }
      else { if (j > 0) j -= 1; else i -= 1; }
      pb[n++] = (j & 1) ? label[(j >> 1) * B + b] : 0;
    }
    s_len = n;
    lens[b] = n;
  }
  __syncthreads();
  const int n = s_len;
  for (int k = threadIdx.x; k < T + LL; k += 256) out[(long long)k * B + b] = (k < n) ? (long long)pb[n - 1 - k] : 0LL;
}

__global__ void gt_counts_kernel(const long long* index_spaced, const int* label, int Tp, int B, int L, float* gt, int* minpos, int* mismatch) {
  const int b = blockIdx.x * blockDim.x + threadIdx.x;
  if (b >= B) return;
  int c = 0, d = 0, pos = 0, last = 0;
  for (int i = 0; i < Tp; ++i) {
    const int index = (int)index_spaced[(long long)i * B + b];
    if (index == 0 && last == 0) c += 1;
    else if (last == 0 || last == index) { d += 1; last = index; }
    else {
      if (pos < L) {
        if (label[pos * B + b] != last) atomicAdd(mismatch, 1);
        gt[((long long)pos * B + b) * 2 + 0] = (float)c;
        gt[((long long)pos * B + b) * 2 + 1] = (float)d;
      } else atomicAdd(mismatch, 1);
      if (index == 0) { c = 1; d = 0; } else { c = 0; d = 1; }
      pos += 1;
      last = index;
    }
  }
  atomicMin(minpos, pos);
}

}

extern "C" int hwg_log_softmax_fwd(const float* x, float* y, long long rows, int C, int B, int T, int transpose_bt, void* stream) {
  HWG_REQUIRE(x && y && rows > 0 && C > 0, "log_softmax_fwd: bad arguments");
  HWG_REQUIRE(!transpose_bt || (long long)B * T == rows, "log_softmax_fwd: B*T != rows");
  long long blocks = (rows + 3) / 4; if (blocks > 2048) blocks = 2048;
  hipLaunchKernelGGL(log_softmax_fwd_kernel, dim3((unsigned)blocks), dim3(256), 0, (hipStream_t)stream, x, y, rows, C, B, T, transpose_bt);
  HWG_LAUNCH_CHECK("log_softmax_fwd");
  return HWG_OK;
}
extern "C" int hwg_log_softmax_bwd(const float* dy, const float* y, float* dx, long long rows, int C, int B, int T, int transpose_bt, void* stream) {
  HWG_REQUIRE(dy && y && dx && rows > 0 && C > 0, "log_softmax_bwd: bad arguments");
  long long blocks = (rows + 3) / 4; if (blocks > 2048) blocks = 2048;
  hipLaunchKernelGGL(log_softmax_bwd_kernel, dim3((unsigned)blocks), dim3(256), 0, (hipStream_t)stream, dy, y, dx, rows, C, B, T, transpose_bt);
  HWG_LAUNCH_CHECK("log_softmax_bwd");
  return HWG_OK;
}

extern "C" size_t hwg_ctc_workspace(int T, int B, int Lmax) {
  const size_t NS = 2 * (size_t)Lmax + 1;
  return (2 * (size_t)B * T * NS + B + 4) * sizeof(float);
}
static int ctc_fwd(const float* log_probs, const int* targets, const int* input_lengths, const int* target_lengths, int T, int B, int C, int Lmax,
                   float* loss, void* ws, size_t ws_bytes, void* stream, bool with_beta) {
  HWG_REQUIRE(log_probs && targets && input_lengths && target_lengths && loss && T > 0 && B > 0 && C > 0 && Lmax > 0, "ctc_fwd: bad arguments");
  if (!ws || ws_bytes < hwg_ctc_workspace(T, B, Lmax)) { hwg_set_error("ctc_fwd: workspace too small"); return HWG_ERR_WORKSPACE; }
  hipStream_t st = (hipStream_t)stream;
  const size_t NS = 2 * (size_t)Lmax + 1;
  float* la = (float*)ws;
  float* lb = la + (size_t)B * T * NS;
  float* nll = lb + (size_t)B * T * NS;
  int* flag = (int*)(nll + B);
  if (with_beta)
    hipLaunchKernelGGL(ctc_alpha_beta_kernel, dim3(2 * B), dim3(256), 3 * NS * sizeof(float), st, log_probs, targets, input_lengths, target_lengths, T, B, C,
                       Lmax, la, nll, lb);
  else
    hipLaunchKernelGGL(ctc_alpha_kernel, dim3(B), dim3(256), 3 * NS * sizeof(float), st, log_probs, targets, input_lengths, target_lengths, T, B, C, Lmax, la, nll);
  HWG_LAUNCH_CHECK("ctc_alpha");
  hipLaunchKernelGGL(ctc_mean_kernel, dim3(1), dim3(64), 0, st, (const float*)nll, target_lengths, B, loss, flag);
  HWG_LAUNCH_CHECK("ctc_mean");
  return HWG_OK;
}
extern "C" int hwg_ctc_fwd(const float* log_probs, const int* targets, const int* input_lengths, const int* target_lengths, int T, int B, int C,
                           int Lmax, float* loss, void* ws, size_t ws_bytes, void* stream) {
  return ctc_fwd(log_probs, targets, input_lengths, target_lengths, T, B, C, Lmax, loss, ws, ws_bytes, stream, false);
}
extern "C" int hwg_ctc_fwd_beta(const float* log_probs, const int* targets, const int* input_lengths, const int* target_lengths, int T, int B, int C,
                                int Lmax, float* loss, void* ws, size_t ws_bytes, void* stream) {
  return ctc_fwd(log_probs, targets, input_lengths, target_lengths, T, B, C, Lmax, loss, ws, ws_bytes, stream, true);
}
static int ctc_bwd(const float* log_probs, const int* targets, const int* input_lengths, const int* target_lengths, int T, int B, int C, int Lmax,
                   const float* grad_out, float* grad, void* ws, size_t ws_bytes, void* stream, bool have_beta) {
  HWG_REQUIRE(log_probs && targets && input_lengths && target_lengths && grad_out && grad, "ctc_bwd: bad arguments");
  if (!ws || ws_bytes < hwg_ctc_workspace(T, B, Lmax)) { hwg_set_error("ctc_bwd: workspace too small"); return HWG_ERR_WORKSPACE; }
  hipStream_t st = (hipStream_t)stream;
  const size_t NS = 2 * (size_t)Lmax + 1;
  float* la = (float*)ws;
  float* lb = la + (size_t)B * T * NS;
  float* nll = lb + (size_t)B * T * NS;
  int* flag = (int*)(nll + B);
  const size_t lds = (2 * NS + NS) * sizeof(float);
  if (!have_beta) {
    hipLaunchKernelGGL(ctc_beta_kernel, dim3(B), dim3(256), lds, st, log_probs, targets, input_lengths, target_lengths, T, B, C, Lmax, lb);
    HWG_LAUNCH_CHECK("ctc_beta");
  }
  hipLaunchKernelGGL(ctc_grad_kernel, dim3(T, B), dim3(128), 2 * NS * sizeof(float), st, log_probs, targets, input_lengths, target_lengths, T, B, C,
                     Lmax, (const float*)la, (const float*)lb, (const float*)nll, grad_out, (const int*)flag, grad);
  HWG_LAUNCH_CHECK("ctc_grad");
  return HWG_OK;
}
extern "C" int hwg_ctc_bwd(const float* log_probs, const int* targets, const int* input_lengths, const int* target_lengths, int T, int B, int C,
                           int Lmax, const float* grad_out, float* grad, void* ws, size_t ws_bytes, void* stream) {
  return ctc_bwd(log_probs, targets, input_lengths, target_lengths, T, B, C, Lmax, grad_out, grad, ws, ws_bytes, stream, false);
}
extern "C" int hwg_ctc_bwd_grad(const float* log_probs, const int* targets, const int* input_lengths, const int* target_lengths, int T, int B, int C,
                                int Lmax, const float* grad_out, float* grad, void* ws, size_t ws_bytes, void* stream) {
  return ctc_bwd(log_probs, targets, input_lengths, target_lengths, T, B, C, Lmax, grad_out, grad, ws, ws_bytes, stream, true);
}

extern "C" size_t hwg_dtw_workspace(int T, int B, int L) {
  const size_t LL = 2 * (size_t)L + 1;
  size_t hist = ((size_t)B * T * LL + 15) / 16 * 16;
  return hist + (size_t)B * (T + LL) * sizeof(int);
}
extern "C" int hwg_dtw_align(const float* pred, const int* label, int T, int B, int C, int L, long long* out, int* lens, void* ws, size_t ws_bytes,
                             void* stream) {
  HWG_REQUIRE(pred && label && out && lens && T > 0 && B > 0 && C > 0 && L > 0, "dtw_align: bad arguments");
  if (!ws || ws_bytes < hwg_dtw_workspace(T, B, L)) { hwg_set_error("dtw_align: workspace too small"); return HWG_ERR_WORKSPACE; }
  const size_t LL = 2 * (size_t)L + 1;
  const size_t hist = ((size_t)B * T * LL + 15) / 16 * 16;
  unsigned char* history = (unsigned char*)ws;
  int* path = (int*)((char*)ws + hist);
  const size_t smem = 3 * (LL + 1) * sizeof(float);
  HWG_REQUIRE(smem <= 64 * 1024, "dtw_align: label too long for LDS (%zu B)", smem);
  hipLaunchKernelGGL(dtw_kernel, dim3(B), dim3(256), smem, (hipStream_t)stream, pred, label, T, B, C, L, history, path, out, lens);
  HWG_LAUNCH_CHECK("dtw_align");
  return HWG_OK;
}

extern "C" int hwg_gt_counts(const long long* index_spaced, const int* label, int Tp, int B, int L, float* gt, int* minpos, int* mismatch,
                             void* stream) {
  HWG_REQUIRE(index_spaced && label && gt && minpos && mismatch && Tp > 0 && B > 0 && L > 0, "gt_counts: bad arguments");
  hipLaunchKernelGGL(gt_counts_kernel, dim3(hwg_cdiv(B, 64)), dim3(64), 0, (hipStream_t)stream, index_spaced, label, Tp, B, L, gt, minpos, mismatch);
  HWG_LAUNCH_CHECK("gt_counts");
  return HWG_OK;
}
```

Before: 91.12.

## Restructure weight packing, wino reduce, CTC and DTW sequence kernels for locality

Mode-0 weight packing now stages a slab of (a,b) pairs times taps in LDS so both global reads and tap-major writes are contiguous. The Winograd balanced-split reduce launches one block per tile and skips tiles with a single owner, instead of grid-striding over every output. CTC alpha/beta gain a single-wave DPP-shift path for short labels and an option to stage emission probabilities in LDS. DTW gets wave/LDS variants, and gt_counts uses one block per batch item with LDS-staged gathers. Together these cut uncoalesced global traffic and barrier costs in small serial kernels, at the price of extra LDS use and more code paths.

```diff
diff --git a/handwriting_line_generation_amd/csrc/conv_mfma.hip b/handwriting_line_generation_amd/csrc/conv_mfma.hip
--- a/handwriting_line_generation_amd/csrc/conv_mfma.hip
+++ b/handwriting_line_generation_amd/csrc/conv_mfma.hip
@@ -893,13 +893,46 @@
 };
 
 constexpr int PACK_PER_BLOCK = 1024;
+constexpr int PACK_SLAB_TAPS = 512;
+constexpr int PACK_SLAB_FLOATS = PACK_PER_BLOCK + 2 * PACK_SLAB_TAPS;
+__device__ __forceinline__ void pack_tap_major_slab(const PackEntry& e, float* dst, long long blk, bool scaled, float sc, float* slab) {
+  const int RS = e.R * e.S;
+  const long long NP = (long long)e.A * e.Bpad;
+  const long long nblk = (e.total + PACK_PER_BLOCK - 1) / PACK_PER_BLOCK;
+  if (blk >= nblk) return;
+  const long long p0 = NP * blk / nblk;
+  const int np = (int)(NP * (blk + 1) / nblk - p0), ld = np | 1;
+  for (int i = threadIdx.x; i < np * RS; i += 256) {
+    const int pair = i / RS, ts = i - pair * RS;
+    const long long p = p0 + pair;
+    const int b = (int)(p % e.Bpad), aa = (int)(p / e.Bpad);
+    const int r = ts / e.S, s2 = ts - r * e.S;
+    float v = 0.f;
+    if (b < e.B) {
+      v = e.src[aa * e.sa + b * e.sb + r * e.sr + s2 * e.ss];
+      if (scaled) v = __fmul_rn(v, sc);
+    }
+    slab[(e.flip ? RS - 1 - ts : ts) * ld + pair] = v;
+  }
+  __syncthreads();
+  for (int i = threadIdx.x; i < np * RS; i += 256) {
+    const int tap = i / np, pair = i - tap * np;
+    dst[tap * NP + p0 + pair] = slab[tap * ld + pair];
+  }
+}
+
 __global__ __launch_bounds__(256) void pack_weight_multi_kernel(const PackEntry* table, int n) {
+  __shared__ float slab[PACK_SLAB_FLOATS];
   int lo = 0, hi = n - 1;
   while (lo < hi) {
     const int mid = (lo + hi + 1) >> 1;
     if (table[mid].first_block <= (long long)blockIdx.x) lo = mid; else hi = mid - 1;
   }
   const PackEntry e = table[lo];
+  if (e.mode == 0 && e.R * e.S <= PACK_SLAB_TAPS) {
+    pack_tap_major_slab(e, e.dst, (long long)blockIdx.x - e.first_block, false, 1.f, slab);
+    return;
+  }
   const long long base = ((long long)blockIdx.x - e.first_block) * PACK_PER_BLOCK;
 #pragma unroll
   for (int j = 0; j < PACK_PER_BLOCK / 256; ++j) {
@@ -929,6 +962,7 @@
   int scale_idx, pad;
 };
 __global__ __launch_bounds__(256) void pack_weight_multi_scaled_kernel(const PackEntryS* table, int n, float* dst_base, const float* scale_base) {
+  __shared__ float slab[PACK_SLAB_FLOATS];
   int lo = 0, hi = n - 1;
   while (lo < hi) {
     const int mid = (lo + hi + 1) >> 1;
@@ -937,6 +971,10 @@
   const PackEntry e = table[lo].e;
   float* dst = dst_base + table[lo].dst_off;
   const float sc = scale_base[table[lo].scale_idx];
+  if (e.mode == 0 && e.R * e.S <= PACK_SLAB_TAPS) {
+    pack_tap_major_slab(e, dst, (long long)blockIdx.x - e.first_block, true, sc, slab);
+    return;
+  }
   const long long base = ((long long)blockIdx.x - e.first_block) * PACK_PER_BLOCK;
 #pragma unroll
   for (int j = 0; j < PACK_PER_BLOCK / 256; ++j) {
diff --git a/handwriting_line_generation_amd/csrc/conv_wino.hip b/handwriting_line_generation_amd/csrc/conv_wino.hip
--- a/handwriting_line_generation_amd/csrc/conv_wino.hip
+++ b/handwriting_line_generation_amd/csrc/conv_wino.hip
@@ -1463,40 +1463,58 @@
 }
 
 template <int VEC>
+__host__ __device__ constexpr int wino_bal_reduce_split(int edge) { return 64 * (64 / VEC) / 256 * edge * edge; }
+template <int VEC>
 __global__ __launch_bounds__(256) void wino_bal_reduce_kernel(WinoK a, int T_all) {
-  const int KV = a.K / VEC;
-  const int total = a.N * a.P * a.Q * KV;
+  const int rel = blockIdx.x;
+  const int U_bal = (a.mt * a.nt - a.bal_tile0) * T_all;
+  const int g_first = wino_bal_owner(a.bal, U_bal, rel * T_all), g_last = wino_bal_owner(a.bal, U_bal, rel * T_all + T_all - 1);
+  if (g_first == g_last) return;
+  constexpr int KL = 64 / VEC;
+  constexpr int ML = 256 / KL;
+  constexpr int MB = 64 / ML;
+  const int tile = a.bal_tile0 + rel, mtile = tile % a.mt, ntile = tile / a.mt;
+  const int k = ntile * 64 + ((int)threadIdx.x % KL) * VEC;
+  const int e = a.mt_edge;
+  const int px = blockIdx.y / MB;
+  const int m = mtile * 64 + ((int)blockIdx.y % MB) * ML + (int)threadIdx.x / KL;
+  if (k >= a.K || m >= a.M) return;
+  const int tj = m % a.TQ, t2 = m / a.TQ, ti = t2 % a.TP, n = t2 / a.TP;
+  const int p = ti * e + px / e, q = tj * e + px % e;
+  if (p >= a.P || q >= a.Q) return;
   const long long plane = (long long)a.N * a.P * a.Q * a.K;
-  const int U_bal = (a.mt * a.nt - a.bal_tile0) * T_all;
-  const int e = a.mt_edge;
-  for (int i = blockIdx.x * blockDim.x + threadIdx.x; i < total; i += gridDim.x * blockDim.x) {
-    const int k = (i % KV) * VEC, pix = i / KV;
-    const int q = pix % a.Q, t = pix / a.Q, p = t % a.P, n = t / a.P;
-    const int m = (n * a.TP + p / e) * a.TQ + q / e;
-    const int rel = (m >> 6) + a.mt * (k >> 6) - a.bal_tile0;
-    if (rel < 0) continue;
-    const int g_first = wino_bal_owner(a.bal, U_bal, rel * T_all), g_last = wino_bal_owner(a.bal, U_bal, rel * T_all + T_all - 1);
-    if (g_first == g_last) continue;
-    const long long o = (long long)n * a.y_img + (long long)p * a.y_row + (long long)q * a.y_pix + (long long)(k / a.y_kc) * a.y_run + k % a.y_kc;
-    float s[VEC];
-#pragma unroll
-    for (int v = 0; v < VEC; ++v) s[v] = 0.f;
-    for (int j = 0; j <= g_last - g_first; ++j) {
+  const long long o = (long long)n * a.y_img + (long long)p * a.y_row + (long long)q * a.y_pix + (long long)(k / a.y_kc) * a.y_run + k % a.y_kc;
+  const float* __restrict__ part = a.part + o;
+  const int pieces = g_last - g_first + 1;
+  float s[VEC];
+#pragma unroll
+  for (int v = 0; v < VEC; ++v) s[v] = 0.f;
+  for (int j0 = 0; j0 < pieces; j0 += 4) {
+    float t[4][VEC];
+#pragma unroll
+    for (int u = 0; u < 4; ++u) {
+      const float* src = part + min(j0 + u, pieces - 1) * plane;
       if constexpr (VEC == 4) {
-        const float4 v = *reinterpret_cast<const float4*>(a.part + j * plane + o);
-        s[0] += v.x; s[1] += v.y; s[2] += v.z; s[3] += v.w;
+        const float4 v = *reinterpret_cast<const float4*>(src);
+        t[u][0] = v.x; t[u][1] = v.y; t[u][2] = v.z; t[u][3] = v.w;
       } else {
-        s[0] += a.part[j * plane + o];
-      }
-    }
-#pragma unroll
-    for (int v = 0; v < VEC; ++v) {
-      if (a.bias) s[v] += a.bias[k + v];
-      if (a.accumulate) s[v] += a.y[o + v];
-    }
-    if constexpr (VEC == 4) *reinterpret_cast<float4*>(a.y + o) = make_float4(s[0], s[1], s[2], s[3]);
-    else a.y[o] = s[0];
-  }
+        t[u][0] = *src;
+      }
+    }
+#pragma unroll
+    for (int u = 0; u < 4; ++u)
+      if (j0 + u < pieces) {
+#pragma unroll
+        for (int v = 0; v < VEC; ++v) s[v] += t[u][v];
+      }
+  }
+#pragma unroll
+  for (int v = 0; v < VEC; ++v) {
+    if (a.bias) s[v] += a.bias[k + v];
+    if (a.accumulate) s[v] += a.y[o + v];
+  }
+  if constexpr (VEC == 4) *reinterpret_cast<float4*>(a.y + o) = make_float4(s[0], s[1], s[2], s[3]);
+  else a.y[o] = s[0];
 }
 
 struct WinoPlan {
@@ -1694,7 +1712,7 @@
     const double cut = (double)(k.mt * k.nt - p.bal_tile0) / (k.mt * k.nt);
     const int prof2 = hwg_prof_open(HWG_PROF_CONV_REDUCE, 4.0 * total * cut * (p.bal_pieces + 1), st);
     const int vec = d->K % 4 == 0 ? 4 : 1;
-    const dim3 rgrid(hwg_stream_grid(total / vec, 256));
+    const dim3 rgrid(k.mt * k.nt - p.bal_tile0, vec == 4 ? wino_bal_reduce_split<4>(2) : wino_bal_reduce_split<1>(2));
     if (vec == 4) hipLaunchKernelGGL(wino_bal_reduce_kernel<4>, rgrid, dim3(256), 0, st, k, d->C / 16);
     else hipLaunchKernelGGL(wino_bal_reduce_kernel<1>, rgrid, dim3(256), 0, st, k, d->C / 16);
     hwg_prof_close(prof2, st);
@@ -1873,7 +1891,7 @@
   } else if (p.bal > 0 && p.bal_pieces > 1) {
     const double cut = (double)(k.mt * k.nt - p.bal_tile0) / (k.mt * k.nt);
     const int prof2 = hwg_prof_open(HWG_PROF_CONV_REDUCE, 4.0 * total * cut * (p.bal_pieces + 1), st);
-    hipLaunchKernelGGL(wino_bal_reduce_kernel<4>, dim3(hwg_stream_grid(total / 4, 256)), dim3(256), 0, st, k, g.Cv / 16);
+    hipLaunchKernelGGL(wino_bal_reduce_kernel<4>, dim3(k.mt * k.nt - p.bal_tile0, wino_bal_reduce_split<4>(3)), dim3(256), 0, st, k, g.Cv / 16);
     hwg_prof_close(prof2, st);
     HWG_LAUNCH_CHECK("wino_bal_reduce");
   } else if (p.bal <= 0 && p.nsplit > 1) {
diff --git a/handwriting_line_generation_amd/csrc/seq_ops.hip b/handwriting_line_generation_amd/csrc/seq_ops.hip
--- a/handwriting_line_generation_amd/csrc/seq_ops.hip
+++ b/handwriting_line_generation_amd/csrc/seq_ops.hip
@@ -39,11 +39,45 @@
   }
 }
 
+__device__ __forceinline__ float wave_shr1(float v, float fill) {
+  return __builtin_bit_cast(float, __builtin_amdgcn_update_dpp(__builtin_bit_cast(int, fill), __builtin_bit_cast(int, v), 0x138, 0xf, 0xf, false));
+}
+__device__ __forceinline__ float wave_shl1(float v, float fill) {
+  return __builtin_bit_cast(float, __builtin_amdgcn_update_dpp(__builtin_bit_cast(int, fill), __builtin_bit_cast(int, v), 0x130, 0xf, 0xf, false));
+}
+
 __device__ __forceinline__ int ctc_ext(const int* tg, int s) { return (s & 1) ? tg[s >> 1] : 0; }
 
-__device__ __forceinline__ void ctc_alpha_body(float* rows , int b, const float* lp,
-                                               const int* targets, const int* in_len, const int* tg_len, int T, int B, int C, int Lmax,
-                                               float* log_alpha, float* nll) {
+enum { CTC_STAGED = 1, CTC_WAVE = 2 };
+constexpr int SEQ_GATHER = 16;
+
+__device__ __forceinline__ float ctc_step(float la1, float la2, float la3, float l) {
+  const float NEG = -INFINITY;
+  float lamax = la1;
+  if (la2 > lamax) lamax = la2;
+  if (la3 > lamax) lamax = la3;
+  if (lamax == NEG) lamax = 0.f;
+  return logf(expf(la1 - lamax) + expf(la2 - lamax) + expf(la3 - lamax)) + lamax + l;
+}
+
+__device__ __forceinline__ void ctc_stage(float* lt, const int* ext, const float* lp, int b, int Tb, int B, int C, int NS, int NSmax) {
+  const int n = Tb * NSmax;
+  for (int base = threadIdx.x; base < n; base += 256 * SEQ_GATHER) {
+    float v[SEQ_GATHER];
+#pragma unroll
+    for (int u = 0; u < SEQ_GATHER; ++u) {
+      const int idx = min(base + u * 256, n - 1), t = idx / NSmax, s = idx - t * NSmax;
+      v[u] = lp[((long long)t * B + b) * C + ext[s]];
+    }
+#pragma unroll
+    for (int u = 0; u < SEQ_GATHER; ++u)
+      if (base + u * 256 < n) lt[base + u * 256] = v[u];
+  }
+}
+
+template <bool STAGED>
+__device__ __forceinline__ void ctc_alpha_body(float* rows, int b, const float* lp, const int* targets, const int* in_len, const int* tg_len, int T,
+                                               int B, int C, int Lmax, float* log_alpha, float* nll, int plan) {
   const int S = tg_len[b];
   const int Tb = in_len[b];
   const int NS = 2 * S + 1;
@@ -51,6 +85,7 @@
   const int* tg = targets + (long long)b * Lmax;
   float* la = log_alpha + (long long)b * T * NSmax;
   int* ext = (int*)(rows + 2 * NSmax);
+  const float* lt = rows + 3 * NSmax;
   const float NEG = -INFINITY;
   for (int s = threadIdx.x; s < NSmax; s += 256) {
     float v = NEG;
@@ -63,31 +98,60 @@
     ext[s] = s < NS ? ctc_ext(tg, s) : 0;
   }
   __syncthreads();
-  for (int t = 1; t < Tb; ++t) {
-    const float* prev = rows + ((t - 1) & 1) * NSmax;
-    float* cur = rows + (t & 1) * NSmax;
-    for (int s = threadIdx.x; s < NSmax; s += 256) {
-      float v = NEG;
-      if (s < NS) {
-        const int cs = ext[s];
-        const float l = lp[((long long)t * B + b) * C + cs];
-        const float la1 = prev[s];
-        float lamax = la1;
-        float la2 = NEG, la3 = NEG;
-        if (s > 0) { la2 = prev[s - 1]; if (la2 > lamax) lamax = la2; }
-        if (s > 1 && ext[s - 2] != cs) { la3 = prev[s - 2]; if (la3 > lamax) lamax = la3; }
-        if (lamax == NEG) lamax = 0.f;
-        v = logf(expf(la1 - lamax) + expf(la2 - lamax) + expf(la3 - lamax)) + lamax + l;
+  if constexpr (STAGED) {
+    ctc_stage(rows + 3 * NSmax, ext, lp, b, Tb, B, C, NS, NSmax);
+    __syncthreads();
+  }
+  auto emit = [&](int t, int s, int cs) {
+    if constexpr (STAGED) return lt[t * NSmax + s];
+    else return lp[((long long)t * B + b) * C + cs];
+  };
+  float r = (S == 0) ? 0.f : INFINITY;
+  if (plan & CTC_WAVE) {
+    if (threadIdx.x >= 64) return;
+    const int s = threadIdx.x;
+    const bool live = s < NS;
+    const int cs = live ? ext[s] : 0;
+    const bool skip = live && s > 1 && ext[s - 2] != cs;
+    float a = s < NSmax ? rows[s] : NEG;
+    float ln = (live && Tb > 1) ? emit(1, s, cs) : 0.f;
+    for (int t = 1; t < Tb; ++t) {
+      const float l = ln;
+      if (live && t + 1 < Tb) ln = emit(t + 1, s, cs);
+      const float p1 = wave_shr1(a, NEG), p2 = wave_shr1(p1, NEG);
+      a = live ? ctc_step(a, s > 0 ? p1 : NEG, skip ? p2 : NEG, l) : NEG;
+      if (s < NSmax) la[(long long)t * NSmax + s] = a;
+    }
+    const float l1 = __shfl(a, NS - 1), l2s = __shfl(a, S > 0 ? NS - 2 : 0);
+    if (Tb > 0) {
+      const float l2 = (S > 0) ? l2s : NEG;
+      float m = fmaxf(l1, l2);
+      if (m == NEG) m = 0.f;
+      r = -(logf(expf(l1 - m) + expf(l2 - m)) + m);
+    }
+  } else {
+    const int s0 = threadIdx.x;
+    const bool live0 = s0 < NS;
+    const int cs0 = live0 ? ext[s0] : 0;
+    float ln = (live0 && Tb > 1) ? emit(1, s0, cs0) : 0.f;
+    for (int t = 1; t < Tb; ++t) {
+      const float* prev = rows + ((t - 1) & 1) * NSmax;
+      float* cur = rows + (t & 1) * NSmax;
+      const float l0 = ln;
+      if (live0 && t + 1 < Tb) ln = emit(t + 1, s0, cs0);
+      for (int s = threadIdx.x; s < NSmax; s += 256) {
+        float v = NEG;
+        if (s < NS) {
+          const int cs = ext[s];
+          const float l = s == s0 ? l0 : emit(t, s, cs);
+          v = ctc_step(prev[s], s > 0 ? prev[s - 1] : NEG, (s > 1 && ext[s - 2] != cs) ? prev[s - 2] : NEG, l);
+        }
+        cur[s] = v;
+        la[(long long)t * NSmax + s] = v;
       }
-      cur[s] = v;
-      la[(long long)t * NSmax + s] = v;
-    }
-    __syncthreads();
-  }
-  if (threadIdx.x == 0) {
-    float r;
-    if (Tb <= 0) r = (S == 0) ? 0.f : INFINITY;
-    else {
+      __syncthreads();
+    }
+    if (Tb > 0) {
       const float* last = rows + ((Tb - 1) & 1) * NSmax;
       const float l1 = last[NS - 1];
       const float l2 = (S > 0) ? last[NS - 2] : NEG;
@@ -95,13 +159,14 @@
       if (m == NEG) m = 0.f;
       r = -(logf(expf(l1 - m) + expf(l2 - m)) + m);
     }
-    nll[b] = r;
-  }
+  }
+  if (threadIdx.x == 0) nll[b] = r;
 }
 __global__ __launch_bounds__(256) void ctc_alpha_kernel(const float* lp, const int* targets, const int* in_len, const int* tg_len, int T, int B,
-                                                        int C, int Lmax, float* log_alpha, float* nll) {
+                                                        int C, int Lmax, float* log_alpha, float* nll, int plan) {
   extern __shared__ float rows[];
-  ctc_alpha_body(rows, blockIdx.x, lp, targets, in_len, tg_len, T, B, C, Lmax, log_alpha, nll);
+  if (plan & CTC_STAGED) ctc_alpha_body<true>(rows, blockIdx.x, lp, targets, in_len, tg_len, T, B, C, Lmax, log_alpha, nll, plan);
+  else ctc_alpha_body<false>(rows, blockIdx.x, lp, targets, in_len, tg_len, T, B, C, Lmax, log_alpha, nll, plan);
 }
 __global__ void ctc_mean_kernel(const float* nll, const int* tg_len, int B, float* loss, int* finite_flag) {
   if (threadIdx.x == 0 && blockIdx.x == 0) {
@@ -113,9 +178,9 @@
     *loss = inf ? 0.f : s;
   }
 }
-__device__ __forceinline__ void ctc_beta_body(float* rows , int b, const float* lp,
-                                              const int* targets, const int* in_len, const int* tg_len, int T, int B, int C, int Lmax,
-                                              float* log_beta) {
+template <bool STAGED>
+__device__ __forceinline__ void ctc_beta_body(float* rows, int b, const float* lp, const int* targets, const int* in_len, const int* tg_len, int T,
+                                              int B, int C, int Lmax, float* log_beta, int plan) {
   const int S = tg_len[b];
   const int Tb = in_len[b];
   const int NS = 2 * S + 1;
@@ -123,28 +188,56 @@
   const int* tg = targets + (long long)b * Lmax;
   float* lb = log_beta + (long long)b * T * NSmax;
   int* ext = (int*)(rows + 2 * NSmax);
+  const float* lt = rows + 3 * NSmax;
   const float NEG = -INFINITY;
   for (int s = threadIdx.x; s < NSmax; s += 256) ext[s] = s < NS ? ctc_ext(tg, s) : 0;
   __syncthreads();
   if (Tb <= 0) return;
+  if constexpr (STAGED) {
+    ctc_stage(rows + 3 * NSmax, ext, lp, b, Tb, B, C, NS, NSmax);
+    __syncthreads();
+  }
+  auto emit = [&](int t, int s, int cs) {
+    if constexpr (STAGED) return lt[t * NSmax + s];
+    else return lp[((long long)t * B + b) * C + cs];
+  };
+  if (plan & CTC_WAVE) {
+    if (threadIdx.x >= 64) return;
+    const int s = threadIdx.x;
+    const bool live = s < NS;
+    const int cs = live ? ext[s] : 0;
+    const bool skip = live && s < NS - 2 && ext[s + 2] != cs;
+    float bv = NEG;
+    if (live && (s == NS - 1 || (S > 0 && s == NS - 2))) bv = emit(Tb - 1, s, cs);
+    if (s < NSmax) lb[(long long)(Tb - 1) * NSmax + s] = bv;
+    float ln = (live && Tb > 1) ? emit(Tb - 2, s, cs) : 0.f;
+    for (int t = Tb - 2; t >= 0; --t) {
+      const float l = ln;
+      if (live && t > 0) ln = emit(t - 1, s, cs);
+      const float n1 = wave_shl1(bv, NEG), n2 = wave_shl1(n1, NEG);
+      bv = live ? ctc_step(bv, s < NS - 1 ? n1 : NEG, skip ? n2 : NEG, l) : NEG;
+      if (s < NSmax) lb[(long long)t * NSmax + s] = bv;
+    }
+    return;
+  }
+  const int s0 = threadIdx.x;
+  const bool live0 = s0 < NS;
+  const int cs0 = live0 ? ext[s0] : 0;
+  float ln = live0 ? emit(Tb - 1, s0, cs0) : 0.f;
   for (int t = Tb - 1; t >= 0; --t) {
     float* cur = rows + (t & 1) * NSmax;
     const float* nxt = rows + ((t + 1) & 1) * NSmax;
+    const float l0 = ln;
+    if (live0 && t > 0) ln = emit(t - 1, s0, cs0);
     for (int s = threadIdx.x; s < NSmax; s += 256) {
       float v = NEG;
       if (s < NS) {
         const int cs = ext[s];
-        const float l = lp[((long long)t * B + b) * C + cs];
+        const float l = s == s0 ? l0 : emit(t, s, cs);
         if (t == Tb - 1) {
           if (s == NS - 1 || (S > 0 && s == NS - 2)) v = l;
         } else {
-          const float lb1 = nxt[s];
-          float lbmax = lb1;
-          float lb2 = NEG, lb3 = NEG;
-          if (s < NS - 1) { lb2 = nxt[s + 1]; if (lb2 > lbmax) lbmax = lb2; }
-          if (s < NS - 2 && ext[s + 2] != cs) { lb3 = nxt[s + 2]; if (lb3 > lbmax) lbmax = lb3; }
-          if (lbmax == NEG) lbmax = 0.f;
-          v = logf(expf(lb1 - lbmax) + expf(lb2 - lbmax) + expf(lb3 - lbmax)) + lbmax + l;
+          v = ctc_step(nxt[s], s < NS - 1 ? nxt[s + 1] : NEG, (s < NS - 2 && ext[s + 2] != cs) ? nxt[s + 2] : NEG, l);
         }
       }
       cur[s] = v;
@@ -154,15 +247,23 @@
   }
 }
 __global__ __launch_bounds__(256) void ctc_beta_kernel(const float* lp, const int* targets, const int* in_len, const int* tg_len, int T, int B,
-                                                       int C, int Lmax, float* log_beta) {
+                                                       int C, int Lmax, float* log_beta, int plan) {
   extern __shared__ float rows[];
-  ctc_beta_body(rows, blockIdx.x, lp, targets, in_len, tg_len, T, B, C, Lmax, log_beta);
+  if (plan & CTC_STAGED) ctc_beta_body<true>(rows, blockIdx.x, lp, targets, in_len, tg_len, T, B, C, Lmax, log_beta, plan);
+  else ctc_beta_body<false>(rows, blockIdx.x, lp, targets, in_len, tg_len, T, B, C, Lmax, log_beta, plan);
 }
 __global__ __launch_bounds__(256) void ctc_alpha_beta_kernel(const float* lp, const int* targets, const int* in_len, const int* tg_len, int T, int B,
-                                                             int C, int Lmax, float* log_alpha, float* nll, float* log_beta) {
+                                                             int C, int Lmax, float* log_alpha, float* nll, float* log_beta, int plan) {
   extern __shared__ float rows[];
-  if ((int)blockIdx.x < B) ctc_alpha_body(rows, blockIdx.x, lp, targets, in_len, tg_len, T, B, C, Lmax, log_alpha, nll);
-  else ctc_beta_body(rows, blockIdx.x - B, lp, targets, in_len, tg_len, T, B, C, Lmax, log_beta);
+  const bool alpha = (int)blockIdx.x < B;
+  const int b = alpha ? blockIdx.x : blockIdx.x - B;
+  if (plan & CTC_STAGED) {
+    if (alpha) ctc_alpha_body<true>(rows, b, lp, targets, in_len, tg_len, T, B, C, Lmax, log_alpha, nll, plan);
+    else ctc_beta_body<true>(rows, b, lp, targets, in_len, tg_len, T, B, C, Lmax, log_beta, plan);
+  } else {
+    if (alpha) ctc_alpha_body<false>(rows, b, lp, targets, in_len, tg_len, T, B, C, Lmax, log_alpha, nll, plan);
+    else ctc_beta_body<false>(rows, b, lp, targets, in_len, tg_len, T, B, C, Lmax, log_beta, plan);
+  }
 }
 
 __global__ __launch_bounds__(128) void ctc_grad_kernel(const float* lp, const int* targets, const int* in_len, const int* tg_len, int T, int B, int C,
@@ -209,8 +310,13 @@
   }
 }
 
+enum { DTW_GLOBAL = 0, DTW_LDS = 1, DTW_WAVE = 2 };
+constexpr int DTW_GATHER = 32;
+
+template <int PLAN>
 __global__ __launch_bounds__(256) void dtw_kernel(const float* pred, const int* label, int T, int B, int C, int L, unsigned char* history,
-                                                  int* path, long long* out, int* lens) {
+                                                  int* path, long long* out, int* lens, int stage_labels) {
+  constexpr bool FULL = PLAN != DTW_GLOBAL;
   extern __shared__ float diag[];
   const int b = blockIdx.x;
   const int LL = 2 * L + 1;
@@ -218,30 +324,83 @@
   float* d0 = diag;
   float* d1 = diag + (LL + 1);
   float* d2 = diag + 2 * (LL + 1);
+  int* labs = (int*)(diag + 3 * (LL + 1));
+  int* pl = labs + LL;
+  float* cost_l = (float*)(pl + (T + LL));
+  unsigned char* hist_l = (unsigned char*)(cost_l + (long long)T * LL);
   const float INF = INFINITY;
-  unsigned char* hist = history + (long long)b * T * LL;
+  unsigned char* hist = FULL ? hist_l : history + (long long)b * T * LL;
+  int* pb = FULL ? pl : path + (long long)b * (T + LL);
+  auto lab_of = [&](int j0) { return (FULL || stage_labels) ? labs[j0] : ((j0 & 1) ? label[(j0 >> 1) * B + b] : 0); };
+  auto in_band = [&](int i, int j) { return i >= 1 && i <= T && j >= 1 && j >= max(1, i - w) && j <= min(LL, i + w); };
   for (int j = threadIdx.x; j <= LL; j += 256) { d0[j] = INF; d1[j] = INF; d2[j] = INF; }
+  if (FULL || stage_labels)
+    for (int j0 = threadIdx.x; j0 < LL; j0 += 256) labs[j0] = (j0 & 1) ? label[(j0 >> 1) * B + b] : 0;
   __syncthreads();
   if (threadIdx.x == 0) d1[0] = 0.f;
+  if constexpr (FULL) {
+    for (int base = threadIdx.x; base < T * LL; base += 256 * DTW_GATHER) {
+      float v[DTW_GATHER];
+#pragma unroll
+      for (int u = 0; u < DTW_GATHER; ++u) {
+        const int idx = min(base + u * 256, T * LL - 1), i0 = idx / LL, j0 = idx - i0 * LL;
+        v[u] = pred[((long long)i0 * B + b) * C + labs[j0]];
+      }
+#pragma unroll
+      for (int u = 0; u < DTW_GATHER; ++u)
+        if (base + u * 256 < T * LL) cost_l[base + u * 256] = 1.f - v[u];
+    }
+  }
   __syncthreads();
-  for (int d = 1; d <= T + LL; ++d) {
+  if constexpr (PLAN == DTW_WAVE) {
+    if (threadIdx.x < 64) {
+      const int j = threadIdx.x;
+      const bool lane_on = j >= 1 && j <= LL;
+      const int d_lo = lane_on ? j + max(1, j - w) : 1, d_hi = lane_on ? j + min(T, j + w) : 0;
+      float cur = j == 0 ? 0.f : INF;
+      float dg = INF;
+      float cn = 0.f;
+      int cell = (1 - j - 1) * LL + (j - 1);
+      for (int d = 1; d <= T + LL; ++d, cell += LL) {
+        const float cost = cn;
+        if (d + 1 >= d_lo && d + 1 <= d_hi) cn = cost_l[cell + LL];
+        const float lf = wave_shr1(cur, INF);
+        float v = INF;
+        if (d >= d_lo && d <= d_hi) {
+          float m = cur; int h = 0;
+          if (dg < m) { m = dg; h = 1; }
+          if (lf < m) { m = lf; h = 2; }
+          v = cost + m;
+          hist_l[cell] = (unsigned char)h;
+        }
+        dg = lf;
+        cur = v;
+      }
+    }
+    __syncthreads();
+  }
+  const int j_own = threadIdx.x;
+  float pn = 0.f;
+  for (int d = 1; PLAN != DTW_WAVE && d <= T + LL; ++d) {
+    const float p_own = pn;
+    if constexpr (!FULL) {
+      if (j_own <= LL && in_band(d + 1 - j_own, j_own)) pn = pred[((long long)(d - j_own) * B + b) * C + lab_of(j_own - 1)];
+    }
     for (int j = threadIdx.x; j <= LL; j += 256) {
       const int i = d - j;
       float v = INF;
-      if (i >= 1 && i <= T && j >= 1) {
-        const int jlo = max(1, i - w), jhi = min(LL, i + w);
-        if (j >= jlo && j <= jhi) {
-          const int lab = ((j - 1) & 1) ? label[((j - 1) >> 1) * B + b] : 0;
-          const float cost = 1.f - pred[((long long)(i - 1) * B + b) * C + lab];
-          const float up = d1[j];
-          const float dg = d0[j - 1];
-          const float lf = d1[j - 1];
-          float m = up; int h = 0;
-          if (dg < m) { m = dg; h = 1; }
-          if (lf < m) { m = lf; h = 2; }
-          v = cost + m;
-          hist[(long long)(i - 1) * LL + (j - 1)] = (unsigned char)h;
-        }
+      if (in_band(i, j)) {
+        float cost;
+        if constexpr (FULL) cost = cost_l[(i - 1) * LL + (j - 1)];
+        else cost = 1.f - (j == j_own ? p_own : pred[((long long)(i - 1) * B + b) * C + lab_of(j - 1)]);
+        const float up = d1[j];
+        const float dg = d0[j - 1];
+        const float lf = d1[j - 1];
+        float m = up; int h = 0;
+        if (dg < m) { m = dg; h = 1; }
+        if (lf < m) { m = lf; h = 2; }
+        v = cost + m;
+        hist[(long long)(i - 1) * LL + (j - 1)] = (unsigned char)h;
       }
       d2[j] = v;
     }
@@ -249,16 +408,15 @@
     float* tmp = d0; d0 = d1; d1 = d2; d2 = tmp;
   }
   __shared__ int s_len;
-  int* pb = path + (long long)b * (T + LL);
   if (threadIdx.x == 0) {
     int i = T - 1, j = LL - 1, n = 0;
-    pb[n++] = (j & 1) ? label[(j >> 1) * B + b] : 0;
+    pb[n++] = lab_of(j);
     while ((i > 0 || j > 0) && n < T + LL) {
       const int h = hist[(long long)i * LL + j];
       if (h == 0) { if (i > 0) i -= 1; else j -= 1; }
       else if (h == 1) { if (i > 0) i -= 1; if (j > 0) j -= 1; }
       else { if (j > 0) j -= 1; else i -= 1; }
-      pb[n++] = (j & 1) ? label[(j >> 1) * B + b] : 0;
+      pb[n++] = lab_of(j);
     }
     s_len = n;
     lens[b] = n;
@@ -268,26 +426,46 @@
   for (int k = threadIdx.x; k < T + LL; k += 256) out[(long long)k * B + b] = (k < n) ? (long long)pb[n - 1 - k] : 0LL;
 }
 
-__global__ void gt_counts_kernel(const long long* index_spaced, const int* label, int Tp, int B, int L, float* gt, int* minpos, int* mismatch) {
-  const int b = blockIdx.x * blockDim.x + threadIdx.x;
-  if (b >= B) return;
+constexpr int GT_BLOCK = 1024;
+__global__ __launch_bounds__(64) void gt_counts_kernel(const long long* index_spaced, const int* label, int Tp, int B, int L, float* gt, int* minpos,
+                                                       int* mismatch) {
+  __shared__ __attribute__((aligned(16))) int col[GT_BLOCK];
+  __shared__ int lab[GT_BLOCK];
+  const int b = blockIdx.x;
+  for (int p = threadIdx.x; p < min(L, GT_BLOCK); p += 64) lab[p] = label[p * B + b];
   int c = 0, d = 0, pos = 0, last = 0;
-  for (int i = 0; i < Tp; ++i) {
-    const int index = (int)index_spaced[(long long)i * B + b];
-    if (index == 0 && last == 0) c += 1;
-    else if (last == 0 || last == index) { d += 1; last = index; }
-    else {
-      if (pos < L) {
-        if (label[pos * B + b] != last) atomicAdd(mismatch, 1);
-        gt[((long long)pos * B + b) * 2 + 0] = (float)c;
-        gt[((long long)pos * B + b) * 2 + 1] = (float)d;
-      } else atomicAdd(mismatch, 1);
-      if (index == 0) { c = 1; d = 0; } else { c = 0; d = 1; }
-      pos += 1;
-      last = index;
-    }
-  }
-  atomicMin(minpos, pos);
+  int4 quad = make_int4(0, 0, 0, 0);
+  for (int i0 = 0; i0 < Tp; i0 += GT_BLOCK) {
+    const int n = min(GT_BLOCK, Tp - i0);
+    __syncthreads();
+    for (int base = threadIdx.x; base < n; base += 64 * SEQ_GATHER) {
+      int v[SEQ_GATHER];
+#pragma unroll
+      for (int u = 0; u < SEQ_GATHER; ++u) v[u] = (int)index_spaced[(long long)(i0 + min(base + u * 64, n - 1)) * B + b];
+#pragma unroll
+      for (int u = 0; u < SEQ_GATHER; ++u)
+        if (base + u * 64 < n) col[base + u * 64] = v[u];
+    }
+    __syncthreads();
+    if (threadIdx.x != 0) continue;
+    for (int i = 0; i < n; ++i) {
+      if ((i & 3) == 0) quad = *reinterpret_cast<const int4*>(col + i);
+      const int index = (i & 3) == 0 ? quad.x : (i & 3) == 1 ? quad.y : (i & 3) == 2 ? quad.z : quad.w;
+      if (index == 0 && last == 0) c += 1;
+      else if (last == 0 || last == index) { d += 1; last = index; }
+      else {
+        if (pos < L) {
+          if ((pos < GT_BLOCK ? lab[pos] : label[pos * B + b]) != last) atomicAdd(mismatch, 1);
+          gt[((long long)pos * B + b) * 2 + 0] = (float)c;
+          gt[((long long)pos * B + b) * 2 + 1] = (float)d;
+        } else atomicAdd(mismatch, 1);
+        if (index == 0) { c = 1; d = 0; } else { c = 0; d = 1; }
+        pos += 1;
+        last = index;
+      }
+    }
+  }
+  if (threadIdx.x == 0) atomicMin(minpos, pos);
 }
 
 }
@@ -311,6 +489,15 @@
 extern "C" size_t hwg_ctc_workspace(int T, int B, int Lmax) {
   const size_t NS = 2 * (size_t)Lmax + 1;
   return (2 * (size_t)B * T * NS + B + 4) * sizeof(float);
+}
+constexpr size_t SEQ_LDS_BUDGET = 64 * 1024;
+static int ctc_plan(int T, int Lmax, size_t* lds) {
+  const size_t NS = 2 * (size_t)Lmax + 1;
+  const size_t base = 3 * NS * sizeof(float), staged = base + (size_t)T * NS * sizeof(float);
+  int plan = NS <= 64 ? CTC_WAVE : 0;
+  if (staged <= SEQ_LDS_BUDGET) plan |= CTC_STAGED;
+  *lds = (plan & CTC_STAGED) ? staged : base;
+  return plan;
 }
 static int ctc_fwd(const float* log_probs, const int* targets, const int* input_lengths, const int* target_lengths, int T, int B, int C, int Lmax,
                    float* loss, void* ws, size_t ws_bytes, void* stream, bool with_beta) {
@@ -322,11 +509,13 @@
   float* lb = la + (size_t)B * T * NS;
   float* nll = lb + (size_t)B * T * NS;
   int* flag = (int*)(nll + B);
+  size_t lds;
+  const int plan = ctc_plan(T, Lmax, &lds);
   if (with_beta)
-    hipLaunchKernelGGL(ctc_alpha_beta_kernel, dim3(2 * B), dim3(256), 3 * NS * sizeof(float), st, log_probs, targets, input_lengths, target_lengths, T, B, C,
-                       Lmax, la, nll, lb);
+    hipLaunchKernelGGL(ctc_alpha_beta_kernel, dim3(2 * B), dim3(256), lds, st, log_probs, targets, input_lengths, target_lengths, T, B, C, Lmax, la, nll,
+                       lb, plan);
   else
-    hipLaunchKernelGGL(ctc_alpha_kernel, dim3(B), dim3(256), 3 * NS * sizeof(float), st, log_probs, targets, input_lengths, target_lengths, T, B, C, Lmax, la, nll);
+    hipLaunchKernelGGL(ctc_alpha_kernel, dim3(B), dim3(256), lds, st, log_probs, targets, input_lengths, target_lengths, T, B, C, Lmax, la, nll, plan);
   HWG_LAUNCH_CHECK("ctc_alpha");
   hipLaunchKernelGGL(ctc_mean_kernel, dim3(1), dim3(64), 0, st, (const float*)nll, target_lengths, B, loss, flag);
   HWG_LAUNCH_CHECK("ctc_mean");
@@ -350,9 +539,10 @@
   float* lb = la + (size_t)B * T * NS;
   float* nll = lb + (size_t)B * T * NS;
   int* flag = (int*)(nll + B);
-  const size_t lds = (2 * NS + NS) * sizeof(float);
   if (!have_beta) {
-    hipLaunchKernelGGL(ctc_beta_kernel, dim3(B), dim3(256), lds, st, log_probs, targets, input_lengths, target_lengths, T, B, C, Lmax, lb);
+    size_t lds;
+    const int plan = ctc_plan(T, Lmax, &lds);
+    hipLaunchKernelGGL(ctc_beta_kernel, dim3(B), dim3(256), lds, st, log_probs, targets, input_lengths, target_lengths, T, B, C, Lmax, lb, plan);
     HWG_LAUNCH_CHECK("ctc_beta");
   }
   hipLaunchKernelGGL(ctc_grad_kernel, dim3(T, B), dim3(128), 2 * NS * sizeof(float), st, log_probs, targets, input_lengths, target_lengths, T, B, C,
@@ -382,9 +572,18 @@
   const size_t hist = ((size_t)B * T * LL + 15) / 16 * 16;
   unsigned char* history = (unsigned char*)ws;
   int* path = (int*)((char*)ws + hist);
-  const size_t smem = 3 * (LL + 1) * sizeof(float);
-  HWG_REQUIRE(smem <= 64 * 1024, "dtw_align: label too long for LDS (%zu B)", smem);
-  hipLaunchKernelGGL(dtw_kernel, dim3(B), dim3(256), smem, (hipStream_t)stream, pred, label, T, B, C, L, history, path, out, lens);
+  const size_t rolling = 3 * (LL + 1) * sizeof(float), labels = LL * sizeof(int);
+  const size_t full = rolling + labels + ((size_t)T + LL) * sizeof(int) + (size_t)T * LL * (sizeof(float) + 1);
+  HWG_REQUIRE(rolling <= SEQ_LDS_BUDGET, "dtw_align: label too long for LDS (%zu B)", rolling);
+  if (full <= SEQ_LDS_BUDGET && LL + 1 <= 64) {
+    hipLaunchKernelGGL(dtw_kernel<DTW_WAVE>, dim3(B), dim3(256), full, (hipStream_t)stream, pred, label, T, B, C, L, history, path, out, lens, 1);
+  } else if (full <= SEQ_LDS_BUDGET) {
+    hipLaunchKernelGGL(dtw_kernel<DTW_LDS>, dim3(B), dim3(256), full, (hipStream_t)stream, pred, label, T, B, C, L, history, path, out, lens, 1);
+  } else {
+    const int stage = rolling + labels <= SEQ_LDS_BUDGET;
+    hipLaunchKernelGGL(dtw_kernel<DTW_GLOBAL>, dim3(B), dim3(256), stage ? rolling + labels : rolling, (hipStream_t)stream, pred, label, T, B, C, L,
+                       history, path, out, lens, stage);
+  }
   HWG_LAUNCH_CHECK("dtw_align");
   return HWG_OK;
 }
@@ -392,7 +591,7 @@
 extern "C" int hwg_gt_counts(const long long* index_spaced, const int* label, int Tp, int B, int L, float* gt, int* minpos, int* mismatch,
                              void* stream) {
   HWG_REQUIRE(index_spaced && label && gt && minpos && mismatch && Tp > 0 && B > 0 && L > 0, "gt_counts: bad arguments");
-  hipLaunchKernelGGL(gt_counts_kernel, dim3(hwg_cdiv(B, 64)), dim3(64), 0, (hipStream_t)stream, index_spaced, label, Tp, B, L, gt, minpos, mismatch);
+  hipLaunchKernelGGL(gt_counts_kernel, dim3(B), dim3(64), 0, (hipStream_t)stream, index_spaced, label, Tp, B, L, gt, minpos, mismatch);
   HWG_LAUNCH_CHECK("gt_counts");
   return HWG_OK;
 }
```

After: 75.77. 16.8% lower.
